# iammadab/zk

Hardware: AMD Instinct MI355X
Metric: field-ops/sec (MLE fold, 2^24 evals, BN254 Fr) + sumcheck prover wall-clock (higher is better)
Workload: dtype u256 (8 x u32 Montgomery limbs, integer)

## Files before the change

zk_amd/csrc/capi.hip:

```cpp
#include <hip/hip_runtime.h>
#include <sched.h>

#include <algorithm>
#include <array>
#include <atomic>
#include <chrono>
#include <condition_variable>
#include <mutex>
#include <cstdio>
#include <map>
#include <new>
#include <set>
#include <string>
#include <thread>
#include <utility>
#include <vector>

#include "../../include/zk_amd.h"
#include "host_core.hpp"
#include "copy_helpers.hpp"
#include "prover_state.hpp"
#include "env.hpp"
#include "kernels.cuh"
#include "eval_kernels.cuh"
// ... 77 lines not shown
        case ZK_ERR_VERIFY_ROUNDS: return "invalid proof: require 1 round poly for each variable in poly";
        case ZK_ERR_VERIFY_SUM: return "verifier check failed: claimed_sum != p(0) + p(1)";
        case ZK_ERR_COEFF_RANGE: return "coefficient map represents more than specificed number of variables";
        case ZK_ERR_PANIC_INVERSE: return "reference panics: (x_i - x_j).inverse().unwrap() on a repeated x (interpolate_xy)";
        case ZK_ERR_EVAL_ASSIGNMENT: return "evaluate requires an assignment for every variable";
        case ZK_ERR_SELECTOR_LEN: return "the selector array len should be the same as the number of variables";
        case ZK_ERR_SELECTOR_SINGLE: return "only select single variable, cannot get indexes for constant or multiple variables";
        case ZK_ERR_BAD_ARG: return "bad argument";
        case ZK_ERR_BAD_FIELD: return "unknown field id";
        case ZK_ERR_NO_DEVICE: return "no usable gfx950 device (libzk_amd has no CPU fallback)";
        case ZK_ERR_HIP: return "HIP runtime error (see zk_last_hip_error)";
        case ZK_ERR_ALLOC: return "allocation failed";
        case ZK_ERR_UNSUPPORTED: return "unsupported configuration";
        case ZK_ERR_CONTEXT_MISMATCH: return "handle belongs to a different context";
        case ZK_ERR_GKR_REJECT: return "gkr verifier check failed: layer wiring / input claim mismatch";
        case ZK_ERR_COMM: return "collective failed (see zk_last_hip_error)";
        default: return "unknown status";
    }
}
extern "C" const char *zk_last_hip_error(void) { return g_hip_err.c_str(); }

extern "C" int32_t zk_device_count(int32_t *out) {
    if (!out) return ZK_ERR_BAD_ARG;
    int n = 0;
    if (hipGetDeviceCount(&n) != hipSuccess) n = 0;
    *out = n;
    return ZK_OK;
}

extern "C" int32_t zk_field_modulus(int32_t field, uint64_t out[4]) {
    const uint64_t *m = field_modulus_limbs(field);
    if (!m || !out) return m ? ZK_ERR_BAD_ARG : ZK_ERR_BAD_FIELD;
    memcpy(out, m, 32);
    return ZK_OK;
}
extern "C" int32_t zk_field_two_adicity(int32_t field, int32_t *out) {
    const FieldInfo *fi = field_info(field);
    if (!fi) return ZK_ERR_BAD_FIELD;
    if (!out) return ZK_ERR_BAD_ARG;
    *out = (int32_t)fi->two_adicity;
    return ZK_OK;
}
extern "C" int32_t zk_field_root_of_unity(int32_t field, uint64_t log_n, uint64_t out[4]) {
    const FieldInfo *fi = field_info(field);
    if (!fi) return ZK_ERR_BAD_FIELD;
    if (!out) return ZK_ERR_BAD_ARG;
    Fe w;
    if (log_n > 64 || !field_root_of_unity(*fi, (uint32_t)log_n, w)) return ZK_ERR_FFT_NO_ROOT;
    fe_to_u64limbs(w, out);
    return ZK_OK;
}
extern "C" int32_t zk_fe_from_u64(int32_t field, uint64_t v, uint64_t out[4]) {
    const FieldInfo *fi = field_info(field);
    if (!fi) return ZK_ERR_BAD_FIELD;
    uint64_t l[4] = {v, 0, 0, 0};
    fe_to_u64limbs(fe_from_canonical(fe_from_u64limbs(l), fi->P), out);
    return ZK_OK;
}
extern "C" int32_t zk_fe_from_canonical(int32_t field, const uint64_t limbs[4], uint64_t out[4]) {
    const FieldInfo *fi = field_info(field);
    if (!fi) return ZK_ERR_BAD_FIELD;
    Fe c = fe_from_u64limbs(limbs), d;
    if (!sub8(d.v, c.v, fi->P.p)) return ZK_ERR_BAD_ARG;
    fe_to_u64limbs(fe_from_canonical(c, fi->P), out);
    return ZK_OK;
}
extern "C" int32_t zk_fe_to_canonical(int32_t field, const uint64_t a[4], uint64_t out[4]) {
    const FieldInfo *fi = field_info(field);
    if (!fi) return ZK_ERR_BAD_FIELD;
    fe_to_u64limbs(fe_to_canonical(fe_from_u64limbs(a), fi->P), out);
    return ZK_OK;
}
extern "C" int32_t zk_fe_from_be_bytes_mod_order(int32_t field, const uint8_t *bytes, size_t len, uint64_t out[4]) {
    const FieldInfo *fi = field_info(field);
    if (!fi) return ZK_ERR_BAD_FIELD;
    fe_to_u64limbs(fe_from_be_bytes_mod_order(bytes, len, fi->P), out);
    return ZK_OK;
}

static int32_t ctx_init_device(zk_ctx *c) {
    HIPCHK(hipSetDevice(c->device));
    HIPCHK(hipStreamCreateWithFlags(&c->own_stream, hipStreamNonBlocking));
    c->stream = c->own_stream;
    HIPCHK(hipMalloc(&c->d_partials, (size_t)kMaxGrid * kMaxSums * 32));
    HIPCHK(hipMalloc(&c->d_sums, (size_t)kMaxSums * 32 * 3));
    HIPCHK(hipHostMalloc(&c->h_pinned, (size_t)kMaxSums * 32 * 3, kPolledHostFlags));
    HIPCHK(hipHostMalloc((void **)&c->h_flag, 64 * kMaxBatch, kPolledHostFlags));
    memset(c->h_flag, 0, 64 * kMaxBatch);
    HIPCHK(hipEventCreate(&c->ev0));
    HIPCHK(hipEventCreate(&c->ev1));
    return ZK_OK;
}
static void ctx_teardown(zk_ctx *c) {
    (void)hipSetDevice(c->device);
    if (c->own_stream) (void)hipStreamSynchronize(c->stream);
    for (auto &kv : c->twiddles) (void)hipFree(kv.second);
    for (auto &kv : c->lagrange_w) (void)hipFree(kv.second);
    for (auto &kv : c->ntt_plans) {
        (void)hipFree((void *)kv.second.w_lo);
        (void)hipFree((void *)kv.second.w_hi);
        for (int p = 0; p < 4; ++p)
            if (kv.second.w_full[p]) (void)hipFree((void *)kv.second.w_full[p]);
    }
    pool_trim(c);
    (void)hipFree(c->d_partials);
    (void)hipFree(c->d_sums);
    if (c->h_pinned) (void)hipHostFree(c->h_pinned);
    if (c->h_flag) (void)hipHostFree(c->h_flag);
    if (c->h_results) (void)hipHostFree(c->h_results);
    for (int b = 0; b < 2; ++b) {
        if (c->h_absorb[b]) (void)hipHostFree(c->h_absorb[b]);
        if (c->ev_absorb[b]) (void)hipEventDestroy(c->ev_absorb[b]);
    }
    if (c->ev0) (void)hipEventDestroy(c->ev0);
    if (c->ev1) (void)hipEventDestroy(c->ev1);
    if (c->own_stream) (void)hipStreamDestroy(c->own_stream);
    delete c;
}
extern "C" int32_t zk_ctx_create(int32_t field, int32_t device, zk_ctx **out) {
    if (!out) return ZK_ERR_BAD_ARG;
    const FieldInfo *fi = field_info(field);
    if (!fi) return ZK_ERR_BAD_FIELD;
    int n = 0;
    if (hipGetDeviceCount(&n) != hipSuccess || n <= 0 || device < 0 || device >= n) return ZK_ERR_NO_DEVICE;
    hipDeviceProp_t prop;
    if (hipGetDeviceProperties(&prop, device) != hipSuccess) return ZK_ERR_NO_DEVICE;
    if (std::string(prop.gcnArchName).find("gfx950") == std::string::npos) return ZK_ERR_NO_DEVICE;
    zk_ctx *c = new (std::nothrow) zk_ctx();
    if (!c) return ZK_ERR_ALLOC;
    c->field = field;
    c->device = device;
    c->fi = fi;
    c->own_stream = c->stream = nullptr;
    c->ev0 = c->ev1 = nullptr;
    c->d_partials = c->d_sums = c->h_pinned = nullptr;
    c->h_flag = nullptr;
    c->flag_seq = 0;
    c->h_results = nullptr;
    c->h_results_bytes = 0;
    c->pool_bytes = c->pool_checked = 0;
    c->inv2 = fe_inverse(fe_from_u32(2, fi->P), fi->P);
    c->pipe_consts.inv2p = mul29_prepare(c->inv2, fi->P);
    {
        Fe v = {{1, 0, 0, 0, 0, 0, 0, 0}};
        for (int i = 0; i < 266; ++i) v = fe_add(v, v, fi->P);
        split29(v.v, c->pipe_consts.k266.l);
    }
    c->d_dbg = nullptr;
    c->dbg_launch = 0;
    c->h_absorb[0] = c->h_absorb[1] = nullptr;
    c->h_absorb_bytes = 0;
    c->ev_absorb[0] = c->ev_absorb[1] = nullptr;
    const int32_t rc = ctx_init_device(c);
    if (rc != ZK_OK) {
        ctx_teardown(c);
        return rc;
    }
    *out = c;
    return ZK_OK;
}
extern "C" int32_t zk_ctx_destroy(zk_ctx *c) {
    if (!c) return ZK_OK;
    ctx_teardown(c);
    return ZK_OK;
}
extern "C" int32_t zk_ctx_synchronize(zk_ctx *c) {
    if (!c) return ZK_ERR_BAD_ARG;
// ... 647 lines not shown
    if (f[0]->ctx != c) return ZK_ERR_CONTEXT_MISMATCH;
    if (k > (uint64_t)kMaxFactors) return ZK_ERR_UNSUPPORTED;
    return use_device(c);
}

extern "C" int32_t zk_prod_reduce(zk_ctx *c, const zk_mle *const *f, uint64_t k, zk_mle **out) {
    if (!out) return ZK_ERR_BAD_ARG;
    ZKCHK(product_args(c, f, k));
    zk_mle *o = nullptr;
    ZKCHK(mle_alloc(c, f[0]->n_vars, &o));
    FactorPtrs fp = {};
    for (uint64_t i = 0; i < k; ++i) fp.in[i] = f[i]->d;
    const uint64_t n = 1ull << f[0]->n_vars;
    if (n >= 64) {
        uint64_t g = n / kBlock;
        if (g > 2 * kMaxGridStream) g = 2 * kMaxGridStream;
        k_prod_reduce_run<<<(uint32_t)(g ? g : 1), kBlock, 0, c->stream>>>(fp, (int)k, n, o->d, c->fi->P);
    } else {
        k_prod_reduce<<<grid_for(n), kBlock, 0, c->stream>>>(fp, (int)k, n, o->d, c->fi->P);
    }
    HIPCHK(hipGetLastError());
    *out = o;
    return ZK_OK;
}

extern "C" int32_t zk_product_evaluate(zk_ctx *c, const zk_mle *const *f, uint64_t k, const uint64_t *point,
                                       uint64_t n_point, uint64_t out[4]) {
    if (!out || (!point && n_point)) return ZK_ERR_BAD_ARG;
    ZKCHK(product_args(c, f, k));
    if (n_point != f[0]->n_vars) return ZK_ERR_EVAL_ARITY;
    Fe prod = fe_one(c->fi->P);
    for (uint64_t i = 0; i < k; ++i) {
        uint64_t v[4];
        ZKCHK(zk_mle_evaluate(c, f[i], point, n_point, v));
        prod = fe_mul(prod, fe_from_u64limbs(v), c->fi->P);
    }
    fe_to_u64limbs(prod, out);
    return ZK_OK;
}

static inline uint64_t *epart_counters(uint64_t *d_epart) { return d_epart + 2 * (kEpartBytes / 8); }
static int32_t scratch_alloc(zk_ctx *c, ProverScratch &ps, uint64_t rounds, uint32_t D, const DeviceChain *chain = nullptr) {
    ps = ProverScratch{};
    ps.rp_bytes = (size_t)(rounds ? rounds : 1) * (D + 1) * 32;
    ps.ch_bytes = (size_t)(rounds ? rounds : 1) * 32;
    if (chain) {
        ps.external = true;
        ps.d_sponge = chain->d_sponge;
        ps.d_rp = chain->d_rp;
        ps.d_ch = chain->d_ch;
        ps.d_final = chain->d_final;
        ps.d_epart = chain->d_epart;
    } else {
        ZKCHK(ps.sponge_block.alloc(c, sizeof(WordSponge)));
        ps.d_sponge = ps.sponge_block.as<WordSponge>();
    }
    ZKCHK(ps.chal_block.alloc(c, kChalBlockBytes));
    ps.d_challenge = ps.chal_block.as();
    ps.d_claim = ps.d_challenge + 2 * kChalWords;
    if (chain) return ZK_OK;
    ZKCHK(ps.epart_block.alloc(c, kEpartBlockBytes));
    ps.d_epart = ps.epart_block.as();
    ZKCHK(ps.proof_block.alloc(c, ps.proof_block_bytes()));
    ps.d_rp = ps.proof_block.as();
    ps.d_ch = ps.d_rp + ps.rp_bytes / 8;
    ps.d_final = ps.d_ch + ps.ch_bytes / 8;
    return ZK_OK;
}
int32_t zk::results_staging(zk_ctx *c, size_t bytes, uint8_t **out) {
    if (c->h_results_bytes < bytes) {
        if (c->h_results) (void)hipHostFree(c->h_results);
        c->h_results = nullptr;
        c->h_results_bytes = 0;
        size_t cap = 1 << 16;
        while (cap < bytes) cap <<= 1;
        HIPCHK(hipHostMalloc((void **)&c->h_results, cap, kPolledHostFlags));
        c->h_results_bytes = cap;
    }
    *out = c->h_results;
    return ZK_OK;
}

static inline uint64_t partials_capacity() { return g_batch ? (uint64_t)kMaxGrid * kMaxSums / kMaxBatch : (uint64_t)kMaxGrid * kMaxSums; }
static inline uint64_t *partials_of(zk_ctx *c) { return g_batch ? c->d_partials + (size_t)g_batch->cur * partials_capacity() * 4 : c->d_partials; }
static inline RoundLaunchCtx launch_ctx(zk_ctx *c) {
    RoundLaunchCtx lc = {c->stream, &c->fi->P, partials_of(c), partials_capacity(), {}};
    return lc;
}
static int32_t launch_tail(zk_ctx *c, uint32_t nblocks, uint32_t ns, WordSponge *sponge, uint64_t *out_rp, uint64_t *out_ch, uint64_t *d_challenge,
                           uint64_t *lanes, const TailDerive &dv, const PendingSponge *init = nullptr) {
    const uint64_t *part = partials_of(c);
    hipStream_t st = c->stream;
    const FieldParams *P = &c->fi->P;
    if (init && init->valid && sponge == init->dst && !lanes && !g_batch) {
        k_round_tail_init<<<1, kBlock, 0, st>>>(part, nblocks, ns, sponge, out_rp, out_ch, d_challenge, *P, dv, init->w, init->zero2);
        HIPCHK(hipGetLastError());
        return ZK_OK;
    }
    if (init && init->valid) {
        k_store_sponge<<<1, 64, 0, st>>>(init->w, init->dst, init->zero2);
        HIPCHK(hipGetLastError());
    }
    auto single = [=]() {
        k_round_tail<<<1, kBlock, 0, st>>>(part, nblocks, ns, sponge, out_rp, out_ch, d_challenge, lanes, *P, dv);
        return hipGetLastError();
    };
    if (!lanes && batch_record(BK_TAIL, 0, 1, kBlock, 0, nblocks, ns, 0, 0, TailSlot{part, sponge, out_rp, out_ch, d_challenge, dv}, single)) return ZK_OK;
    HIPCHK(single());
    return ZK_OK;
}
int32_t zk::launch_reduce_tail(zk_ctx *c, uint32_t nblocks, uint32_t ns, uint64_t *out_rp) {
    k_round_tail<<<1, kBlock, 0, c->stream>>>(c->d_partials, nblocks, ns, nullptr, out_rp, nullptr, nullptr, nullptr, c->fi->P);
    HIPCHK(hipGetLastError());
    return ZK_OK;
}
static bool claim_in_round() {
    static const bool v = env_u64("ZK_CLAIM_IN_ROUND", 1, 0, 1) != 0;
    return v;
}
static inline bool fast_degree(uint32_t D) { return D >= 1 && D <= 4; }

struct TailTargets {
    WordSponge *sponge;
    uint64_t *out_rp;
    uint64_t *out_ch;
    uint64_t *d_challenge;
    uint64_t *lanes;
    const PendingSponge *init;
    uint64_t *claim_park;
    TailDerive *lanes_dv;
};
static std::vector<Fe> interp_weights_compute(uint32_t D, const FieldParams &P) {
    std::vector<Fe> w(D + 1);
    for (uint32_t i = 0; i <= D; ++i) {
        Fe den = fe_one(P);
        const Fe xi = fe_from_u32(i, P);
        for (uint32_t j = 0; j <= D; ++j)
            if (j != i) den = fe_mul(den, fe_sub(xi, fe_from_u32(j, P), P), P);
        w[i] = fe_inverse(den, P);
    }
    return w;
}
static std::vector<Fe> interp_weights(uint32_t D, const FieldParams &P) {
    static std::mutex mu;
    static std::map<std::pair<std::array<uint32_t, 8>, uint32_t>, std::vector<Fe>> cache;
    std::array<uint32_t, 8> key;
    for (int i = 0; i < 8; ++i) key[i] = P.p[i];
    std::lock_guard<std::mutex> lock(mu);
    auto it = cache.find({key, D});
    if (it == cache.end()) it = cache.emplace(std::make_pair(key, D), interp_weights_compute(D, P)).first;
    return it->second;
}
static uint64_t skip1_min_pairs() {
    static const uint64_t v = env_u64("ZK_SKIP1_MIN_PAIRS", (uint64_t)1 << 16, 1, (uint64_t)1 << 40);
    return v;
}
static inline TermSpec single_term(int k) {
    TermSpec ts = {1, {k, 0, 0, 0}};
    return ts;
}
struct DeferredTail {
    uint32_t blocks;
    bool skip1;
    bool lead;
    const uint64_t *claim;
};
static uint64_t lead_min_pairs() {
    static const uint64_t v = env_u64("ZK_LEAD_MIN_PAIRS", (uint64_t)1 << 16, 1, (uint64_t)1 << 40);
    return v;
}
static bool shard_skip_on() {
    static const bool v = env_u64("ZK_SHARD_SKIP1", 1, 0, 1) != 0;
    return v;
}
static int32_t launch_sums(zk_ctx *c, const FactorPtrs &fp, const TermSpec &ts, uint64_t q, uint32_t D, bool fused,
                           const uint64_t *d_r, const TailTargets &tt, const TailDerive *dv = nullptr, DeferredTail *defer = nullptr) {
    if (defer) defer->blocks = 0;
    const FieldParams &P = c->fi->P;
    if (fast_degree(D)) {
        uint32_t total = 0;
        int first = 0;
        const bool may_derive = !tt.lanes || (tt.lanes_dv && shard_skip_on());
        bool skip1 = dv && dv->prev_rp && tt.claim_park && fused && may_derive && D <= (uint32_t)kMaxSkipDegree && q >= skip1_min_pairs();
        bool lead = may_derive && q >= lead_min_pairs();
        ClaimJob cjob = {};
        if (skip1 && claim_in_round()) cjob = ClaimJob{dv->prev_rp, dv->prev_chal, dv->w, tt.claim_park, D + 1};
        auto with_claim = [&](RoundLaunchCtx lc) {
            lc.claim = cjob;
            return lc;
        };
        auto tail_dv = [&]() {
            TailDerive t = skip1 && dv ? *dv : TailDerive{};
            t.lead = lead ? D : 0;
            t.claim = (t.prev_rp && cjob.out) ? cjob.out : nullptr;
            if (tt.lanes) {
                if (tt.lanes_dv) *tt.lanes_dv = t;
                t.local_only = 1;
            }
            return t;
        };
        if (tt.lanes_dv) *tt.lanes_dv = TailDerive{};
        if (ts.n_terms == 2 && ts.term_k[1] == 1) {
            uint32_t g = 0;
            const int lrc = launch_round_plus1(with_claim(launch_ctx(c)), fp, ts.term_k[0], q, D, fused, d_r, &g, &skip1, &lead);
            if (lrc == kLaunchHipError) {
                g_hip_err = "round kernel launch failed";
                return ZK_ERR_HIP;
            }
            if (lrc == kLaunchOk) {
                if (defer) {
                    defer->blocks = g;
                    defer->skip1 = skip1;
                    defer->claim = skip1 ? cjob.out : nullptr;
                    defer->lead = lead;
                    return ZK_OK;
                }
                return launch_tail(c, g, D + 1, tt.sponge, tt.out_rp, tt.out_ch, tt.d_challenge, tt.lanes, tail_dv(), tt.init);
            }
        }
        if (ts.n_terms != 1) {
            skip1 = lead = false;
            cjob = {};
        }
        for (int i = 0; i < ts.n_terms; ++i) {
            FactorPtrs sub = {};
            for (int f = 0; f < ts.term_k[i]; ++f) {
                sub.in[f] = fp.in[first + f];
                sub.out[f] = fp.out[first + f];
            }
            RoundLaunchCtx lc = with_claim(launch_ctx(c));
            lc.d_partials += (size_t)total * (D + 1) * 4;
            lc.capacity_elems -= (uint64_t)total * (D + 1);
            uint32_t g = 0;
            const int lrc = launch_round(lc, sub, ts.term_k[i], q, D, fused, d_r, &g, &skip1, &lead);
            if (lrc == kLaunchUnsupported) return ZK_ERR_UNSUPPORTED;
            if (lrc != kLaunchOk) {
                g_hip_err = "round kernel launch failed";
                return ZK_ERR_HIP;
            }
            total += g;
            first += ts.term_k[i];
        }
        if (defer) {
            defer->blocks = total;
            defer->skip1 = skip1;
            defer->claim = skip1 ? cjob.out : nullptr;
            defer->lead = lead;
            return ZK_OK;
        }
        return launch_tail(c, total, D + 1, tt.sponge, tt.out_rp, tt.out_ch, tt.d_challenge, tt.lanes, tail_dv(), tt.init);
    }
    if (ts.n_terms != 1) return ZK_ERR_UNSUPPORTED;
    const int k = ts.term_k[0];
    for (uint32_t t = 0; t <= D; ++t) {
        uint32_t g = 0;
        if (launch_round_single_t(launch_ctx(c), fp, k, q, fe_from_u32(t, P), &g) != kLaunchOk) {
            g_hip_err = "round kernel launch failed";
            return ZK_ERR_HIP;
        }
        k_round_tail<<<1, kBlock, 0, c->stream>>>(c->d_partials, g, 1, nullptr, c->d_sums + 4 * t, nullptr, nullptr, nullptr, P);
        HIPCHK(hipGetLastError());
    }
    k_round_tail<<<1, kBlock, 0, c->stream>>>(c->d_sums, 1, D + 1, tt.sponge, tt.out_rp, tt.out_ch, tt.d_challenge, tt.lanes, P);
    HIPCHK(hipGetLastError());
    return ZK_OK;
}

extern "C" int32_t zk_round_sums(zk_ctx *c, const zk_mle *const *f, uint64_t k, uint32_t D, uint64_t *out) {
    if (!out) return ZK_ERR_BAD_ARG;
    ZKCHK(product_args(c, f, k));
    if (D >= kMaxSums) return ZK_ERR_UNSUPPORTED;
    if (f[0]->n_vars == 0) return ZK_ERR_PANIC_INDEX;
    FactorPtrs fp = {};
    for (uint64_t i = 0; i < k; ++i) fp.in[i] = f[i]->d;
    const uint64_t q = 1ull << (f[0]->n_vars - 1);
    uint64_t *d_out = c->d_sums + 4 * kMaxSums;
    TailTargets tt = {nullptr, d_out, nullptr, nullptr, nullptr, nullptr, nullptr};
    ZKCHK(launch_sums(c, fp, single_term((int)k), q, D, false, nullptr, tt));
    HIPCHK(hipMemcpyAsync(out, d_out, (size_t)(D + 1) * 32, hipMemcpyDeviceToHost, c->stream));
    HIPCHK(hipStreamSynchronize(c->stream));
    return ZK_OK;
}

extern "C" int32_t zk_transcript_new(zk_transcript **out) {
    if (!out) return ZK_ERR_BAD_ARG;
    zk_transcript *t = new (std::nothrow) zk_transcript();
    if (!t) return ZK_ERR_ALLOC;
    t->sp.init();
    *out = t;
    return ZK_OK;
}
extern "C" int32_t zk_transcript_free(zk_transcript *t) {
    delete t;
    return ZK_OK;
}
extern "C" int32_t zk_transcript_append(zk_transcript *t, const uint8_t *data, size_t len) {
    if (!t || (!data && len)) return ZK_ERR_BAD_ARG;
    t->sp.update(data, len);
    return ZK_OK;
}
extern "C" int32_t zk_transcript_sample_challenge(zk_transcript *t, uint8_t out[32]) {
    if (!t || !out) return ZK_ERR_BAD_ARG;
    t->sp.sample_challenge(out);
    return ZK_OK;
}
extern "C" int32_t zk_transcript_sample_field_element(zk_transcript *t, int32_t field, uint64_t out[4]) {
    if (!t || !out) return ZK_ERR_BAD_ARG;
    const FieldInfo *fi = field_info(field);
    if (!fi) return ZK_ERR_BAD_FIELD;
    uint8_t h[32];
    t->sp.sample_challenge(h);
    fe_to_u64limbs(fe_from_be_bytes_mod_order(h, 32, fi->P), out);
    return ZK_OK;
}
extern "C" int32_t zk_transcript_sample_n_field_elements(zk_transcript *t, int32_t field, uint64_t n, uint64_t *out) {
    if (!t || (!out && n)) return ZK_ERR_BAD_ARG;
    if (!field_info(field)) return ZK_ERR_BAD_FIELD;
    for (uint64_t i = 0; i < n; ++i) ZKCHK(zk_transcript_sample_field_element(t, field, out + 4 * i));
    return ZK_OK;
}
extern "C" int32_t zk_keccak256(const uint8_t *data, size_t len, uint8_t out[32]) {
    if ((!data && len) || !out) return ZK_ERR_BAD_ARG;
    Sponge s;
    s.init();
    s.update(data, len);
    s.finalize_reset(out);
    return ZK_OK;
}

void zk::absorb_elements(Sponge &sp, const uint64_t *elems, uint64_t n, const FieldParams &P) {
// ... 225 lines not shown
    int k, extra;
    if (!pipe_limit_pairs() || !pipe_shape(st, &k, &extra)) return false;
    if (m_s < 3) return false;
    if (!finish_pipe_on() && m_s - 1 <= (uint64_t)kFinishVars) return false;
    return ((uint64_t)1 << (m_s - 2)) <= pipe_limit_pairs();
}
static int32_t finish_pipe_enqueue(RoundState &st) {
    zk_ctx *c = st.c;
    int k = 0, extra = 0;
    (void)pipe_shape(st, &k, &extra);
    FinishPipeLaunch fl = {};
    fl.k = k;
    fl.extra = extra;
    fl.D = st.D;
    fl.m_in = (uint32_t)st.vars_left;
    fl.entry = st.pipe_active ? 2 : (st.pending_fold ? 1 : 0);
    fl.e_partials = epart_of_round(st, st.round);
    fl.e_blocks = 1;
    if (st.pipe_active && !st.pipe_total) {
        fl.e_partials += (size_t)pipe_values_per_block(k, st.D) * 4;
        fl.e_blocks = st.pipe_blocks;
    }
    fl.pc = c->pipe_consts;
    fl.chal_in = chal_prev(st);
    const uint64_t remaining = st.pending_fold ? st.vars_left - 1 : st.vars_left;
    fl.chal_last = chal_of_round(st, st.round + remaining - 1);
    fl.sponge = st.ps.d_sponge;
    fl.out_rp = st.ps.d_rp + st.round * (st.D + 1) * 4;
    fl.out_ch = st.ps.d_ch + st.round * 4;
    fl.out_final = st.d_final;
    fl.dbg = pipe_dbg_slot(c, true);
    fl.pub = st.pub;
    FactorPtrs fp = {};
    for (uint64_t i = 0; i < st.k; ++i) fp.in[i] = st.cur[i];
    const int lrc = launch_finish_pipe(launch_ctx(c), fp, fl);
    if (lrc != kLaunchOk) {
        g_hip_err = "pipelined finisher launch failed";
        return lrc == kLaunchUnsupported ? ZK_ERR_UNSUPPORTED : ZK_ERR_HIP;
    }
    st.round += remaining;
    st.vars_left = 0;
    st.pending_fold = false;
    st.pipe_active = false;
    st.published = st.pub.flag != nullptr;
    return ZK_OK;
}
static PipeTailArgs pipe_tail_args(const RoundState &st, int mode, const uint64_t *partials, uint32_t nblocks, uint32_t n_in) {
    PipeTailArgs ta = {};
    ta.dbg = pipe_dbg_slot(st.c, false);
    ta.partials = partials;
    ta.nblocks = nblocks;
    ta.n_in = n_in;
    ta.mode = mode;
    ta.chal_in = chal_prev(st);
    ta.chal_out = chal_cur(st);
    ta.sponge = st.ps.d_sponge;
    ta.out_rp = st.ps.d_rp + st.round * (st.D + 1) * 4;
    ta.out_ch = st.ps.d_ch + st.round * 4;
    ta.pc = st.c->pipe_consts;
    return ta;
}
static int32_t pipe_enter(RoundState &st, const DeferredTail &dt) {
    zk_ctx *c = st.c;
    int k = 0, extra = 0;
    (void)pipe_shape(st, &k, &extra);
    PipeLaunch pl = {};
    pl.k = k;
    pl.extra = extra;
    pl.D = st.D;
    pl.fold = false;
    pl.emit = 1;
    pl.q = (uint64_t)1 << (st.vars_left - 2);
    pl.chal_fold = nullptr;
    pl.e_partials = epart_of_round(st, st.round + 1);
    pl.done_counter = epart_counter(st, st.round + 1);
    pl.tail = pipe_tail_args(st, 0, partials_of(c), dt.blocks, st.D + 1);
    if (dt.skip1) {
        pl.tail.dv = st.dv;
        pl.tail.dv.prev_rp = pl.tail.out_rp - (size_t)(st.D + 1) * 4;
        pl.tail.dv.prev_chal = chal_prev(st);
        pl.tail.dv.claim = dt.claim;
    }
    pl.tail.dv.lead = dt.lead ? st.D : 0;
    FactorPtrs fp = {};
    for (uint64_t i = 0; i < st.k; ++i) fp.in[i] = fp.out[i] = st.cur[i];
    uint32_t g = 0;
    const int lrc = launch_round_pipe(launch_ctx(c), fp, pl, &g);
    if (lrc != kLaunchOk) {
        g_hip_err = "pipelined round launch failed";
        return lrc == kLaunchUnsupported ? ZK_ERR_UNSUPPORTED : ZK_ERR_HIP;
    }
    st.pipe_active = true;
    st.pipe_blocks = g;
    st.pipe_total = true;
    return ZK_OK;
}
static int32_t pipe_step(RoundState &st) {
    zk_ctx *c = st.c;
    int k = 0, extra = 0;
    (void)pipe_shape(st, &k, &extra);
    const uint64_t m = st.vars_left;
    const bool stay = pipe_wants_next(st, m - 1);
    PipeLaunch pl = {};
    pl.k = k;
    pl.extra = extra;
    pl.D = st.D;
    pl.fold = true;
    pl.emit = stay ? 1 : 0;
    pl.q = m >= 3 ? (uint64_t)1 << (m - 3) : 0;
    if (pl.q == 0) return ZK_ERR_BAD_ARG;
    pl.chal_fold = chal_prev(st);
    pl.e_partials = epart_of_round(st, st.round + 1);
    pl.done_counter = epart_counter(st, st.round + 1);
    pl.tail = pipe_tail_args(st, 1, epart_of_round(st, st.round), 1, pipe_values_per_block(k, st.D));
    if (!st.pipe_total) {
        pl.tail.partials = epart_of_round(st, st.round) + (size_t)pipe_values_per_block(k, st.D) * 4;
        pl.tail.nblocks = st.pipe_blocks;
    }
    FactorPtrs fp = {};
    for (uint64_t i = 0; i < st.k; ++i) {
        fp.in[i] = st.cur[i];
        fp.out[i] = (st.first_out_of_place && st.scratch[i]) ? st.scratch[i].as() : st.cur[i];
    }
    uint32_t g = 0;
    const int lrc = launch_round_pipe(launch_ctx(c), fp, pl, &g);
    if (lrc != kLaunchOk) {
        g_hip_err = "pipelined round launch failed";
        return lrc == kLaunchUnsupported ? ZK_ERR_UNSUPPORTED : ZK_ERR_HIP;
    }
    for (uint64_t i = 0; i < st.k; ++i) st.cur[i] = fp.out[i];
    st.first_out_of_place = false;
    st.vars_left = m - 1;
    st.pipe_active = stay;
    st.pipe_blocks = g;
    st.pipe_total = true;
    ++st.round;
    return ZK_OK;
}

template <int K, int D>
static int32_t launch_finish(zk_ctx *c, const FactorPtrs &fp, uint32_t m_in, int pending, uint64_t *d_challenge, WordSponge *sp,
                             uint64_t *out_rp, uint64_t *out_ch, uint64_t *out_final) {
    const uint32_t m = pending ? m_in - 1 : m_in;
    const size_t lds = (size_t)K * ((size_t)32 << m) + (kBlock / 64) * (D + 1) * 32 + (D + 1) * 32 + 48;
    HIPCHK(hipFuncSetAttribute(reinterpret_cast<const void *>(&k_finish<K, D>), hipFuncAttributeMaxDynamicSharedMemorySize, (int)lds));
    hipStream_t st = c->stream;
    const FieldParams *P = &c->fi->P;
    auto single = [=]() {
        k_finish<K, D><<<1, kBlock, lds, st>>>(fp, m_in, pending, *P, d_challenge, sp, out_rp, out_ch, out_final);
        return hipGetLastError();
    };
    if (batch_record_other(single)) return ZK_OK;
    HIPCHK(single());
    return ZK_OK;
}
static bool finish_shape_ok(uint64_t k, uint32_t D) {
    const int shape = (int)k * 10 + (int)D;
    return shape == 11 || shape == 12 || shape == 21 || shape == 22 || shape == 23 || shape == 32 || shape == 33;
}
static int32_t finish_enqueue(RoundState &st) {
    zk_ctx *c = st.c;
    FactorPtrs fp = {};
    for (uint64_t i = 0; i < st.k; ++i) fp.in[i] = st.cur[i];
    const int pending = st.pending_fold ? 1 : 0;
    const uint32_t m_in = (uint32_t)st.vars_left;
    const uint64_t remaining = pending ? st.vars_left - 1 : st.vars_left;
    uint64_t *out_rp = st.ps.d_rp + st.round * (st.D + 1) * 4, *out_ch = st.ps.d_ch + st.round * 4;
    int32_t rc = ZK_ERR_UNSUPPORTED;
    if (st.terms.n_terms > 1) {
        const uint32_t m = pending ? m_in - 1 : m_in;
        const size_t lds = (size_t)st.k * ((size_t)32 << m) + (kBlock / 64) * (st.D + 1) * 32 + (st.D + 1) * 32 + 48;
        const FieldParams &P = c->fi->P;
#define ZK_FINISH_TERMS(DD)                                                                                                     \
    case DD:                                                                                                                    \
        if (hipFuncSetAttribute(reinterpret_cast<const void *>(&k_finish_terms<DD>), hipFuncAttributeMaxDynamicSharedMemorySize, \
                                (int)lds) != hipSuccess)                                                                        \
            return ZK_ERR_HIP;                                                                                                  \
        k_finish_terms<DD><<<1, kBlock, lds, c->stream>>>(fp, st.terms, m_in, pending, P, chal_prev(st), st.ps.d_sponge,     \
                                                          out_rp, out_ch, st.d_final);                                          \
        break;
        switch (st.D) {
            ZK_FINISH_TERMS(1)
            ZK_FINISH_TERMS(2)
            ZK_FINISH_TERMS(3)
            ZK_FINISH_TERMS(4)
            default: return ZK_ERR_UNSUPPORTED;
        }
#undef ZK_FINISH_TERMS
        rc = hipGetLastError() == hipSuccess ? ZK_OK : ZK_ERR_HIP;
    } else {
        switch ((int)st.k * 10 + (int)st.D) {
            case 11: rc = launch_finish<1, 1>(c, fp, m_in, pending, chal_prev(st), st.ps.d_sponge, out_rp, out_ch, st.d_final); break;
            case 12: rc = launch_finish<1, 2>(c, fp, m_in, pending, chal_prev(st), st.ps.d_sponge, out_rp, out_ch, st.d_final); break;
            case 21: rc = launch_finish<2, 1>(c, fp, m_in, pending, chal_prev(st), st.ps.d_sponge, out_rp, out_ch, st.d_final); break;
            case 22: rc = launch_finish<2, 2>(c, fp, m_in, pending, chal_prev(st), st.ps.d_sponge, out_rp, out_ch, st.d_final); break;
            case 23: rc = launch_finish<2, 3>(c, fp, m_in, pending, chal_prev(st), st.ps.d_sponge, out_rp, out_ch, st.d_final); break;
            case 32: rc = launch_finish<3, 2>(c, fp, m_in, pending, chal_prev(st), st.ps.d_sponge, out_rp, out_ch, st.d_final); break;
            case 33: rc = launch_finish<3, 3>(c, fp, m_in, pending, chal_prev(st), st.ps.d_sponge, out_rp, out_ch, st.d_final); break;
            default: break;
        }
    }
    if (rc == ZK_OK) {
        st.round += remaining;
        st.vars_left = 0;
        st.pending_fold = false;
    }
    return rc;
}
static inline bool finish_applies(const RoundState &st) {
    if (st.terms.n_terms == 1 ? !finish_shape_ok(st.k, st.D) : !fast_degree(st.D)) return false;
    const uint64_t after = st.pending_fold ? st.vars_left - 1 : st.vars_left;
    return after >= 1 && after <= (uint64_t)kFinishVars;
}

static int32_t prover_step(RoundState &st, bool *finished_in_kernel) {
    if (st.init.valid && (finish_pipe_applies(st) || st.pipe_active || finish_applies(st))) ZKCHK(flush_pending_sponge(st));
    if (finish_pipe_applies(st)) {
        *finished_in_kernel = true;
        return finish_pipe_enqueue(st);
    }
    if (st.pipe_active) return pipe_step(st);
    if (finish_applies(st)) {
        *finished_in_kernel = true;
        return finish_enqueue(st);
    }
    const uint64_t m_s = st.pending_fold ? st.vars_left - 1 : st.vars_left;
    DeferredTail dt = {0, false, false, nullptr};
    const bool enter = fast_degree(st.D) && pipe_wants_next(st, m_s);
    ZKCHK(round_enqueue(st, nullptr, enter ? &dt : nullptr));
    if (enter && dt.blocks) ZKCHK(pipe_enter(st, dt));
    ++st.round;
    return ZK_OK;
}

int32_t zk::sponge_to_device(zk_ctx *c, const Sponge &host, WordSponge *d_sponge, uint64_t *d_epart) {
    WordSponge w;
    if (!w.from_byte_sponge(host)) return ZK_ERR_BAD_ARG;
    uint64_t *zero2 = d_epart ? epart_counters(d_epart) : nullptr;
    hipStream_t st = c->stream;
    auto single = [=]() {
        k_store_sponge<<<1, 64, 0, st>>>(w, d_sponge, zero2);
        return hipGetLastError();
    };
    if (batch_record(BK_STORE_SPONGE, 0, 1, 64, 0, 0, 0, 0, 0, SpongeSlot{w, d_sponge, zero2}, single)) return ZK_OK;
    HIPCHK(single());
    return ZK_OK;
}

static bool has_duplicate_handles(zk_mle *const *f, uint64_t k) {
    for (uint64_t i = 0; i < k; ++i)
        for (uint64_t j = i + 1; j < k; ++j)
            if (f[i] == f[j]) return true;
    return false;
}
int32_t zk::prove_core(zk_ctx *c, zk_mle *const *f, uint64_t k, const TermSpec &ts, uint32_t D, const uint64_t sum[4],
                          int32_t absorb_table, int32_t consume, uint64_t *out_rp, uint64_t *out_ch, uint64_t *out_final,
                          uint64_t *d_keep_ch, uint64_t *d_keep_final, const Sponge *init, const DeviceChain *chain) {
    if (!sum && !chain) return ZK_ERR_BAD_ARG;
    ZKCHK(product_args(c, (const zk_mle *const *)f, k));
    if (chain) {
        const uint64_t n = f[0]->n_vars;
        if (n == 0 || D >= kMaxSums) return ZK_ERR_UNSUPPORTED;
        if (has_duplicate_handles(f, k)) consume = 0;
        RoundState st;
        ZKCHK(round_state_init(st, c, f, k, D, consume != 0, n, chain));
        st.terms = ts;
        st.d_final = st.ps.d_final;
        bool fin = false;
        while (st.round < n) ZKCHK(prover_step(st, &fin));
        if (!fin) {
            FactorPtrs fp = {};
            for (uint64_t i = 0; i < k; ++i) fp.in[i] = st.cur[i];
            k_final_evals<<<1, 64, 0, c->stream>>>(fp, (uint32_t)k, chal_prev(st), st.d_final, c->fi->P);
            HIPCHK(hipGetLastError());
        }
        return ZK_OK;
    }
    if (f[0]->n_vars && (!out_rp || !out_ch)) return ZK_ERR_BAD_ARG;
    if (D >= kMaxSums) return ZK_ERR_UNSUPPORTED;
    const FieldParams &P = c->fi->P;
    const uint64_t n = f[0]->n_vars;
    Sponge sp;
    if (init) sp = *init;
    else sp.init();
    if (absorb_table) ZKCHK(absorb_tables(c, sp, f, k));
    absorb_elements(sp, sum, 1, P);
    if (n == 0) {
        if (out_final)
            for (uint64_t i = 0; i < k; ++i) ZKCHK(zk_mle_download(c, f[i], out_final + 4 * i));
        return ZK_OK;
    }
    if (has_duplicate_handles(f, k)) consume = 0;
    static const bool host_dbg = env_flag("ZK_HOST_DEBUG");
    const auto t_enter = std::chrono::steady_clock::now();
    RoundState st;
    ZKCHK(round_state_init(st, c, f, k, D, consume != 0, n));
    st.terms = ts;
    if (out_final) st.d_final = st.ps.d_final;
    uint8_t *stage = nullptr;
    const size_t block = st.ps.proof_block_bytes();
    uint32_t seq = 0;
    auto enqueue = [&]() -> int32_t {
        static const bool sponge_in_tail = env_u64("ZK_SPONGE_IN_TAIL", 1, 0, 1) != 0;
        if (sponge_in_tail && !g_batch) {
            if (!st.init.w.from_byte_sponge(sp)) return ZK_ERR_BAD_ARG;
            st.init.dst = st.ps.d_sponge;
            st.init.zero2 = st.ps.d_epart ? epart_counters(st.ps.d_epart) : nullptr;
            st.init.valid = true;
        } else {
            ZKCHK(sponge_to_device(c, sp, st.ps.d_sponge, st.ps.d_epart));
// ... 670 lines not shown
```

zk_amd/csrc/common.cuh:

```cuda
#pragma once
#include "field.cuh"

namespace zk {

constexpr int kBlock = 256;
constexpr int kMaxFactors = 8;

struct FactorPtrs {
    const uint64_t *in[kMaxFactors];
    uint64_t *out[kMaxFactors];
};

constexpr int kMaxBatch = 8;
template <class Slot>
struct BatchOf {
    Slot a[kMaxBatch];
};
struct FactorPtrs4 {
    const uint64_t *in[4];
    uint64_t *out[4];
};
ZK_HD FactorPtrs4 factor_ptrs4(const FactorPtrs &f) {
    FactorPtrs4 r;
    for (int i = 0; i < 4; ++i) r.in[i] = f.in[i], r.out[i] = f.out[i];
// ... 11 lines not shown
struct TermSpec {
    int n_terms;
    int term_k[kMaxTerms];
};
#if defined(__HIPCC__)
ZK_D Mul29 load_challenge29c(const uint64_t *rptr) {
    const uint32_t *w = reinterpret_cast<const uint32_t *>(rptr) + kChalCanonWord;
    Mul29 r;
#pragma unroll
    for (int i = 0; i < 9; ++i) r.l[i] = __builtin_amdgcn_readfirstlane(w[i]);
    return r;
}
ZK_D Mul29 load_challenge29(const uint64_t *rptr) {
    const uint32_t *w = reinterpret_cast<const uint32_t *>(rptr) + 8;
    Mul29 r;
#pragma unroll
    for (int i = 0; i < 9; ++i) r.l[i] = __builtin_amdgcn_readfirstlane(w[i]);
    return r;
}
typedef uint32_t u32x4_t __attribute__((ext_vector_type(4)));
ZK_D uint4 nt_load16(const uint4 *p) {
    const u32x4_t v = __builtin_nontemporal_load(reinterpret_cast<const u32x4_t *>(p));
    return make_uint4(v.x, v.y, v.z, v.w);
}
ZK_D void nt_store16(uint4 v, uint4 *p) {
    const u32x4_t w = {v.x, v.y, v.z, v.w};
    __builtin_nontemporal_store(w, reinterpret_cast<u32x4_t *>(p));
}
ZK_D uint32_t swap_pair_lane(uint32_t v) { return __builtin_amdgcn_mov_dpp(v, 0xB1 , 0xF, 0xF, true); }
ZK_D Fe pair_gather(const uint4 &A, const uint4 &B, bool odd) {
    const uint4 send = odd ? A : B;
    const uint4 recv = make_uint4(swap_pair_lane(send.x), swap_pair_lane(send.y), swap_pair_lane(send.z), swap_pair_lane(send.w));
    Fe r;
    if (!odd) r = {{A.x, A.y, A.z, A.w, recv.x, recv.y, recv.z, recv.w}};
    else r = {{recv.x, recv.y, recv.z, recv.w, B.x, B.y, B.z, B.w}};
    return r;
}
ZK_D void pair_scatter(const Fe &e, bool odd, uint4 &A, uint4 &B) {
    const uint4 lo = make_uint4(e.v[0], e.v[1], e.v[2], e.v[3]), hi = make_uint4(e.v[4], e.v[5], e.v[6], e.v[7]);
    const uint4 send = odd ? lo : hi;
    const uint4 recv = make_uint4(swap_pair_lane(send.x), swap_pair_lane(send.y), swap_pair_lane(send.z), swap_pair_lane(send.w));
    if (!odd) {
        A = lo;
        B = recv;
    } else {
        A = recv;
        B = hi;
    }
}
ZK_D uint32_t pair_owned(uint32_t lane) { return (lane >> 1) + ((lane & 1) << 5); }
ZK_D Fe run_load(const uint64_t *run , uint32_t lane) {
    const uint4 *p = reinterpret_cast<const uint4 *>(run) + lane;
    return pair_gather(p[0], p[64], lane & 1);
}
ZK_D void run_store(uint64_t *run, uint32_t lane, const Fe &e) {
    uint4 A, B;
    pair_scatter(e, lane & 1, A, B);
    uint4 *p = reinterpret_cast<uint4 *>(run) + lane;
    p[0] = A;
    p[64] = B;
}

ZK_D Fe run_load_nt(const uint64_t *run, uint32_t lane) {
    const uint4 *p = reinterpret_cast<const uint4 *>(run) + lane;
    return pair_gather(nt_load16(p), nt_load16(p + 64), lane & 1);
}
ZK_D void run_store_nt(uint64_t *run, uint32_t lane, const Fe &e) {
    uint4 A, B;
    pair_scatter(e, lane & 1, A, B);
    uint4 *p = reinterpret_cast<uint4 *>(run) + lane;
    nt_store16(A, p);
    nt_store16(B, p + 64);
}

constexpr int kMaxSkipDegree = 4;
struct TailDerive {
    const uint64_t *prev_rp;
    const uint64_t *prev_chal;
    const uint64_t *w;
    uint32_t lead;
    uint32_t local_only;
    const uint64_t *claim;
    uint32_t log_world;
};
struct ClaimJob {
    const uint64_t *prev_rp;
    const uint64_t *prev_chal;
    const uint64_t *w;
    uint64_t *out;
    uint32_t ns;
};
ZK_HD Fe lead_rebuild(uint32_t D, const Fe *S, const FieldParams &P) {
    const Fe L = S[D];
    if (D == 1) return fe_add(S[0], L, P);
    if (D == 2) {
        const Fe a = fe_add(S[1], L, P);
        return fe_sub(fe_add(a, a, P), S[0], P);
    }
    Fe b = fe_add(fe_sub(S[2], S[1], P), fe_add(L, L, P), P);
    b = fe_add(fe_add(b, b, P), b, P);
    return fe_add(S[0], b, P);
}

template <int CTRL>
ZK_D Fe fe_dpp(const Fe &s) {
    Fe o;
#pragma unroll
    for (int i = 0; i < 8; ++i) o.v[i] = __builtin_amdgcn_update_dpp(0u, s.v[i], CTRL, 0xF, 0xF, true);
    return o;
}
ZK_D Fe fe_wave_sum(Fe s, const FieldParams &P, uint32_t width = 64) {
    if (width > 32) {
        Fe a, b;
#pragma unroll
        for (int i = 0; i < 8; ++i) {
            const auto r = __builtin_amdgcn_permlane32_swap(s.v[i], s.v[i], false, false);
            a.v[i] = r[0];
            b.v[i] = r[1];
        }
        s = fe_add(a, b, P);
    }
    if (width > 16) {
        Fe a, b;
#pragma unroll
        for (int i = 0; i < 8; ++i) {
            const auto r = __builtin_amdgcn_permlane16_swap(s.v[i], s.v[i], false, false);
            a.v[i] = r[0];
            b.v[i] = r[1];
        }
        s = fe_add(a, b, P);
    }
    if (width > 8) s = fe_add(s, fe_dpp<0x128>(s), P);
    if (width > 4) s = fe_add(s, fe_dpp<0x12C>(s), P);
    if (width > 2) s = fe_add(s, fe_dpp<0x12E>(s), P);
    if (width > 1) s = fe_add(s, fe_dpp<0x12F>(s), P);
    return s;
}
ZK_D Fe claim_eval(const ClaimJob &cj, const FieldParams &P) {
    const uint32_t lane = threadIdx.x & 63;
    const Fe r = fe_load(cj.prev_chal, 0);
    Fe term = fe_zero();
    if (lane < cj.ns) {
        Fe one;
#pragma unroll
        for (int i = 0; i < 8; ++i) one.v[i] = P.r1[i];
        term = fe_mul(fe_load(cj.prev_rp, lane), fe_load(cj.w, lane), P);
        Fe node = fe_zero();
        for (uint32_t u = 0; u < cj.ns; ++u) {
            if (u != lane) term = fe_mul(term, fe_sub(r, node, P), P);
            node = fe_add(node, one, P);
        }
    }
    return fe_wave_sum(term, P, 8);
}

constexpr int kEvalHighMax = 12;
struct EvalHighPoint {
    uint32_t n;
    uint32_t r[kEvalHighMax][8];
};
ZK_D uint32_t eval_high_lane(uint32_t n) { return n > 8 ? 15u : n > 4 ? 7u : n > 2 ? 3u : n > 1 ? 1u : 0u; }
ZK_D Fe eval_high_weight(const EvalHighPoint &ph, uint64_t g, uint32_t lane, const FieldParams &P) {
    Fe one;
#pragma unroll
    for (int i = 0; i < 8; ++i) one.v[i] = P.r1[i];
    Fe f = one;
    for (uint32_t k = 0; k < ph.n; ++k) {
        Fe r;
#pragma unroll
        for (int i = 0; i < 8; ++i) r.v[i] = ph.r[k][i];
        const Fe sel = (g >> k) & 1 ? r : fe_sub(one, r, P);
        if ((lane & 15) == k) f = sel;
    }
    if (ph.n > 8) f = fe_mul(f, fe_dpp<0x128>(f), P);
    if (ph.n > 4) f = fe_mul(f, fe_dpp<0x124>(f), P);
    if (ph.n > 2) f = fe_mul(f, fe_dpp<0x122>(f), P);
    if (ph.n > 1) f = fe_mul(f, fe_dpp<0x121>(f), P);
    return f;
}
#endif

}
```

zk_amd/csrc/field.cuh:

```cuda
#pragma once
#include <stdint.h>

#if defined(__HIPCC__)
#include <hip/hip_runtime.h>
#define ZK_HD __host__ __device__ __forceinline__
#define ZK_D __device__ __forceinline__
#else
#define ZK_HD inline
#define ZK_D inline
#endif

namespace zk {

struct FieldParams {
    uint32_t p[8];
    uint32_t r1[8];
    uint32_t r2[8];
    uint32_t inv;
    uint32_t bits;
    uint32_t p29[9];
    uint32_t inv29;
    uint32_t r2_29[9];
    uint32_t r2s_29[9];
};
// ... 275 lines not shown
    return fe_mul(x, r2, P);
}
ZK_HD Fe fe_to_canonical(const Fe &a, const FieldParams &P) {
    uint32_t t[16];
#pragma unroll
    for (int i = 0; i < 8; ++i) {
        t[i] = a.v[i];
        t[i + 8] = 0;
    }
    return redc(t, P);
}
ZK_HD Fe fe_from_u32(uint32_t x, const FieldParams &P) {
    Fe v = {{x, 0, 0, 0, 0, 0, 0, 0}};
    return fe_from_canonical(v, P);
}

template <int KMAX>
ZK_HD void ladder9(uint32_t s[9], const FieldParams &P) {
#pragma unroll
    for (int k = KMAX; k >= 0; --k) {
        uint32_t d[9];
        uint32_t borrow = 0;
#pragma unroll
        for (int i = 0; i < 9; ++i) {
            uint32_t pk;
            if (k == 0) pk = (i < 8) ? P.p[i] : 0u;
            else pk = ((i < 8) ? (P.p[i] << k) : 0u) | ((i > 0) ? (P.p[i - 1] >> (32 - k)) : 0u);
            uint32_t bo;
            d[i] = __builtin_subc(s[i], pk, borrow, &bo);
            borrow = bo;
        }
#pragma unroll
        for (int i = 0; i < 9; ++i) s[i] = borrow ? s[i] : d[i];
    }
}

struct WideAcc {
    uint32_t v[17];
};
ZK_HD void wide_zero(WideAcc &w) {
#pragma unroll
    for (int i = 0; i < 17; ++i) w.v[i] = 0;
}
template <int C>
ZK_HD void wide_mac_col(WideAcc &w, Acc &acc, const uint32_t a[8], const uint32_t b[8]) {
    constexpr int lo = C < 8 ? 0 : C - 7, hi = C < 8 ? C : 7;
    acc_add32(acc, w.v[C]);
    mac_col<hi - lo + 1>(acc, a + lo, b + (C - lo));
    w.v[C] = acc_shift(acc);
    if constexpr (C + 1 < 15) wide_mac_col<C + 1>(w, acc, a, b);
}
ZK_HD void wide_mac(WideAcc &w, const uint32_t a[8], const uint32_t b[8]) {
    Acc acc = {0, 0};
    wide_mac_col<0>(w, acc, a, b);
    acc_add32(acc, w.v[15]);
    w.v[15] = acc_shift(acc);
    w.v[16] += (uint32_t)acc.lh;
}
constexpr int kMaxLazy = 32;
ZK_HD Fe redc_wide(const WideAcc &w, const FieldParams &P) {
    uint32_t m[8];
    Acc acc = {0, 0};
    uint32_t s[9];
    redc_cols<0>(w.v, m, s, acc, P);
    s[8] = (uint32_t)acc.lh;
    {
        uint64_t c = 0;
        const uint32_t top = w.v[16];
#pragma unroll
        for (int i = 0; i < 8; ++i) {
            c += (uint64_t)top * P.r1[i] + s[i];
            s[i] = (uint32_t)c;
            c >>= 32;
        }
        s[8] += (uint32_t)c;
    }
    ladder9<4>(s, P);
    Fe r;
#pragma unroll
    for (int i = 0; i < 8; ++i) r.v[i] = s[i];
    return r;
}

ZK_HD Fe fe_reduce_u256(const uint32_t x[8], const FieldParams &P) {
    uint32_t s[9];
#pragma unroll
    for (int i = 0; i < 8; ++i) s[i] = x[i];
    s[8] = 0;
    ladder9<4>(s, P);
    Fe r;
#pragma unroll
    for (int i = 0; i < 8; ++i) r.v[i] = s[i];
    return r;
}

struct Mul29 {
    uint32_t l[9];
};
ZK_HD void split29(const uint32_t a[8], uint32_t out[9]) {
    constexpr uint32_t M = (1u << 29) - 1;
#pragma unroll
    for (int i = 0; i < 9; ++i) {
        const int bit = 29 * i, w = bit >> 5, sh = bit & 31;
        uint32_t v = a[w] >> sh;
        if (sh > 3 && w + 1 < 8) v |= a[w + 1] << (32 - sh);
        out[i] = (i < 8) ? (v & M) : v;
    }
}
ZK_HD Mul29 mul29_prepare(const Fe &c, const FieldParams &P) {
    Fe t = c;
#pragma unroll
    for (int i = 0; i < 5; ++i) t = fe_add(t, t, P);
    Mul29 m;
    split29(t.v, m.l);
    return m;
}
template <bool LAZY = false, bool TWO = false>
ZK_HD Fe mul29_core(const uint32_t (&x)[9], const uint32_t (&y)[9], const Mul29 &c, const FieldParams &P, const Mul29 *c2 = nullptr) {
    constexpr uint32_t M = (1u << 29) - 1;
    uint32_t m[9], r[9];
    uint64_t acc = 0;
#pragma unroll
    for (int k = 0; k < 9; ++k) {
#pragma unroll
        for (int i = 0; i <= k; ++i) acc += (uint64_t)x[i] * c.l[k - i];
        if constexpr (TWO) {
#pragma unroll
            for (int i = 0; i <= k; ++i) acc += (uint64_t)y[i] * c2->l[k - i];
        }
#pragma unroll
        for (int i = 0; i < k; ++i) acc += (uint64_t)m[i] * P.p29[k - i];
        m[k] = ((uint32_t)acc * P.inv29) & M;
        acc += (uint64_t)m[k] * P.p29[0];
        acc >>= 29;
    }
#pragma unroll
    for (int k = 9; k < 17; ++k) {
#pragma unroll
        for (int i = k - 8; i < 9; ++i) acc += (uint64_t)x[i] * c.l[k - i];
        if constexpr (TWO) {
#pragma unroll
            for (int i = k - 8; i < 9; ++i) acc += (uint64_t)y[i] * c2->l[k - i];
        }
#pragma unroll
        for (int i = k - 8; i < 9; ++i) acc += (uint64_t)m[i] * P.p29[k - i];
        r[k - 9] = (uint32_t)acc & M;
        acc >>= 29;
    }
    r[8] = (uint32_t)acc;
    Fe s;
#pragma unroll
    for (int w = 0; w < 8; ++w) {
        const int bit = 32 * w, i = bit / 29, sh = bit - 29 * i;
        uint32_t v = r[i] >> sh;
        v |= r[i + 1] << (29 - sh);
        if (29 - sh + 29 < 32 && i + 2 < 9) v |= r[i + 2] << (58 - sh);
        s.v[w] = v;
    }
    if constexpr (LAZY) return s;
    Fe d, o;
    const uint32_t borrow = sub8(d.v, s.v, P.p);
#pragma unroll
    for (int i = 0; i < 8; ++i) o.v[i] = borrow ? s.v[i] : d.v[i];
    return o;
}
template <bool LAZY = false, bool TWO = false>
// ... 45 lines not shown
```

zk_amd/csrc/host_field.hpp:

```cpp
#pragma once
#include <stdint.h>
#include <string.h>

#include "field.cuh"

namespace zk {

struct FieldInfo {
    FieldParams P;
    uint32_t two_adicity;
    uint32_t generator;
    Fe two_adic_root;
    bool ready;
};

inline const uint64_t *field_modulus_limbs(int field) {
    static const uint64_t M[3][4] = {
        {0x43e1f593f0000001ULL, 0x2833e84879b97091ULL, 0xb85045b68181585dULL, 0x30644e72e131a029ULL},
        {0xffffffff00000001ULL, 0x53bda402fffe5bfeULL, 0x3339d80809a1d805ULL, 0x73eda753299d7d48ULL},
        {0x0a11800000000001ULL, 0x59aa76fed0000001ULL, 0x60b44d1e5c37b001ULL, 0x12ab655e9a2ca556ULL},
    };
    return (field >= 0 && field < 3) ? M[field] : nullptr;
}

inline Fe fe_from_u64limbs(const uint64_t l[4]) {
    Fe r;
    for (int i = 0; i < 4; ++i) {
        r.v[2 * i] = (uint32_t)l[i];
        r.v[2 * i + 1] = (uint32_t)(l[i] >> 32);
    }
    return r;
}
inline void fe_to_u64limbs(const Fe &a, uint64_t l[4]) {
    for (int i = 0; i < 4; ++i) l[i] = (uint64_t)a.v[2 * i] | ((uint64_t)a.v[2 * i + 1] << 32);
}

inline Fe fe_pow_limbs(const Fe &x, const uint32_t e[8], const FieldParams &P) {
    Fe acc = fe_one(P);
    for (int i = 255; i >= 0; --i) {
        acc = fe_sqr(acc, P);
        if ((e[i / 32] >> (i % 32)) & 1u) acc = fe_mul(acc, x, P);
    }
    return acc;
}
inline Fe fe_pow_u64(const Fe &x, uint64_t e, const FieldParams &P) {
    Fe acc = fe_one(P), base = x;
    while (e) {
        if (e & 1) acc = fe_mul(acc, base, P);
        base = fe_sqr(base, P);
        e >>= 1;
    }
    return acc;
}
inline Fe fe_inverse(const Fe &a, const FieldParams &P) {
    uint32_t e[8], two[8] = {2, 0, 0, 0, 0, 0, 0, 0};
    sub8(e, P.p, two);
    return fe_pow_limbs(a, e, P);
}

inline const FieldInfo *field_info(int field) {
    static FieldInfo info[3];
    static const uint32_t adicity[3] = {28, 32, 47};
    static const uint32_t gen[3] = {5, 7, 22};
    if (field < 0 || field > 2) return nullptr;
    FieldInfo &I = info[field];
    if (I.ready) return &I;
    FieldParams &P = I.P;
    Fe pm = fe_from_u64limbs(field_modulus_limbs(field));
    memcpy(P.p, pm.v, 32);
    uint32_t x = 1;
    for (int i = 0; i < 5; ++i) x *= 2u - P.p[0] * x;
    P.inv = 0u - x;
    int top = 7;
    while (top > 0 && P.p[top] == 0) --top;
    P.bits = 32 * top + (32 - __builtin_clz(P.p[top]));
    uint32_t v[8] = {1, 0, 0, 0, 0, 0, 0, 0}, d[8];
    for (int i = 0; i < 512; ++i) {
        uint32_t c = add8(v, v, v);
        uint32_t b = sub8(d, v, P.p);
        if (c | (b ^ 1u)) memcpy(v, d, 32);
        if (i == 255) memcpy(P.r1, v, 32);
    }
    memcpy(P.r2, v, 32);
    split29(P.p, P.p29);
    P.inv29 = P.inv & ((1u << 29) - 1);
    {
        Fe r2;
        memcpy(r2.v, P.r2, 32);
        const Mul29 k0 = mul29_prepare(r2, P);
        Fe r2s = r2;
        for (int i = 0; i < 5; ++i) r2s = fe_add(r2s, r2s, P);
        const Mul29 k1 = mul29_prepare(r2s, P);
        memcpy(P.r2_29, k0.l, sizeof k0.l);
        memcpy(P.r2s_29, k1.l, sizeof k1.l);
    }
    {
        const int rp_log = 257 - (int)P.bits;
        int lazy_log = 0;
        while ((1 << lazy_log) < kMaxLazy) ++lazy_log;
        const int top_log = lazy_log + 2 * (int)P.bits - 512;
        const uint64_t rp = rp_log >= 0 && rp_log < 32 ? (1ull << rp_log) : ~0ull;
        const uint64_t top = top_log < 0 ? 0 : (top_log < 32 ? (1ull << top_log) : ~0ull);
        if (rp_log < 0 || rp + 1 + top >= 32 || rp + 1 + top < rp) return nullptr;
    }
    I.two_adicity = adicity[field];
    I.generator = gen[field];
    uint32_t t[8], one[8] = {1, 0, 0, 0, 0, 0, 0, 0};
    sub8(t, P.p, one);
    for (uint32_t s = 0; s < I.two_adicity; ++s) {
        for (int i = 0; i < 7; ++i) t[i] = (t[i] >> 1) | (t[i + 1] << 31);
        t[7] >>= 1;
    }
    I.two_adic_root = fe_pow_limbs(fe_from_u32(I.generator, P), t, P);
    I.ready = true;
    return &I;
}

inline bool field_root_of_unity(const FieldInfo &I, uint32_t log_n, Fe &out) {
    if (log_n > I.two_adicity) return false;
    Fe w = I.two_adic_root;
    for (uint32_t i = log_n; i < I.two_adicity; ++i) w = fe_sqr(w, I.P);
    out = w;
    return true;
}

inline void fe_to_bytes_be(const Fe &a, const FieldParams &P, uint8_t out[32]) {
    Fe c = fe_to_canonical(a, P);
    for (int i = 0; i < 8; ++i)
        for (int b = 0; b < 4; ++b) out[31 - (4 * i + b)] = (uint8_t)(c.v[i] >> (8 * b));
}
inline Fe fe_from_be_bytes_mod_order(const uint8_t *bytes, size_t len, const FieldParams &P) {
    Fe acc = fe_zero();
    const Fe c256 = fe_from_u32(256, P);
    for (size_t i = 0; i < len; ++i) acc = fe_add(fe_mul(acc, c256, P), fe_from_u32(bytes[i], P), P);
    return acc;
}

}
```

zk_amd/csrc/kernels.cuh:

```cuda
#pragma once
#include "common.cuh"
#include "keccak.hpp"
#include "transcript.cuh"

namespace zk {

ZK_D uint64_t insert_zero_bit(uint64_t val, uint32_t pos) {
    const uint64_t low = val & ((1ull << pos) - 1ull);
    return ((val >> pos) << (pos + 1)) | low;
}

__global__ __launch_bounds__(kBlock) void k_fold(const uint64_t *in, uint64_t *out,
                                                 uint64_t pairs, uint32_t pos, FieldParams P, Mul29 r) {
    const uint64_t stride = (uint64_t)gridDim.x * kBlock;
    for (uint64_t j = (uint64_t)blockIdx.x * kBlock + threadIdx.x; j < pairs; j += stride) {
        const uint64_t l = insert_zero_bit(j, pos);
        const Fe lo = fe_load(in, l);
        const Fe hi = fe_load(in, l | (1ull << pos));
        const Fe d = fe_sub(lo, hi, P);
        fe_store(out, j, fe_sub(lo, fe_mul29(d, r, P), P));
    }
}

__global__ __launch_bounds__(kBlock) void k_fold_msb(const uint64_t *in, uint64_t *out, uint64_t half, FieldParams P, Mul29 r) {
// ... 256 lines not shown
    }
}

__global__ __launch_bounds__(kBlock) void k_prod_reduce_run(FactorPtrs fp, int k, uint64_t n, uint64_t *__restrict__ out, FieldParams P) {
    const uint32_t lane = threadIdx.x & 63;
    const bool odd = lane & 1;
    const uint64_t wave = ((uint64_t)blockIdx.x * kBlock + threadIdx.x) >> 6;
    const uint64_t nwaves = ((uint64_t)gridDim.x * kBlock) >> 6;
    uint4 *out4 = reinterpret_cast<uint4 *>(out);
    for (uint64_t e0 = wave * 64; e0 < n; e0 += nwaves * 64) {
        const uint64_t c0 = 2 * e0 + lane;
        Fe acc;
        {
            const uint4 *q = reinterpret_cast<const uint4 *>(fp.in[0]);
            acc = pair_gather(nt_load16(q + c0), nt_load16(q + c0 + 64), odd);
        }
        for (int f = 1; f < k; ++f) {
            const uint4 *q = reinterpret_cast<const uint4 *>(fp.in[f]);
            acc = fe_mul_tt(acc, pair_gather(nt_load16(q + c0), nt_load16(q + c0 + 64), odd), P);
        }
        uint4 oa, ob;
        pair_scatter(acc, odd, oa, ob);
        nt_store16(oa, out4 + c0);
        nt_store16(ob, out4 + c0 + 64);
    }
}
__global__ __launch_bounds__(kBlock) void k_prod_reduce(FactorPtrs fp, int k, uint64_t n, uint64_t *__restrict__ out,
                                                        FieldParams P) {
    const uint64_t stride = (uint64_t)gridDim.x * kBlock;
    for (uint64_t j = (uint64_t)blockIdx.x * kBlock + threadIdx.x; j < n; j += stride) {
        Fe acc = fe_load(fp.in[0], j);
        for (int f = 1; f < k; ++f) acc = fe_mul(acc, fe_load(fp.in[f], j), P);
        fe_store(out, j, acc);
    }
}

ZK_D LaneSponge lane_sponge_from_arg(const WordSponge &w, const LaneKeccak &L) {
    LaneSponge sp;
    sp.a = 0;
#pragma unroll
    for (int i = 0; i < 25; ++i)
        if (L.index == i) sp.a = w.s[i];
    sp.pos = w.pos;
    return sp;
}
ZK_D void round_tail_body(const uint64_t *__restrict__ partials, uint32_t nblocks, uint32_t ns, WordSponge *__restrict__ sponge,
                          uint64_t *__restrict__ out_rp, uint64_t *__restrict__ out_ch, uint64_t *__restrict__ d_challenge,
                          uint64_t *__restrict__ lanes, const FieldParams &P, const TailDerive &dv, const WordSponge *init = nullptr,
                          uint64_t *__restrict__ zero2 = nullptr) {
    __shared__ Fe fin[256];
    __shared__ Fe claim;
    const int lane = threadIdx.x & 63, wave = threadIdx.x >> 6;
    const bool wave0 = __builtin_amdgcn_readfirstlane(wave) == 0;
    const bool derive1 = dv.prev_rp != nullptr;
    const LaneKeccak L = lane_keccak_init();
    LaneSponge sp = {0, 0};
    if (sponge && wave0) sp = init ? lane_sponge_from_arg(*init, L) : lane_sponge_load(sponge, L);
    if (init && zero2 && threadIdx.x >= 64 && threadIdx.x < 66) zero2[threadIdx.x - 64] = 0;
    for (uint32_t t = wave; t < ns; t += kBlock / 64) {
        if (derive1 && t == 1 && (dv.claim || dv.local_only)) {
            if (lane == 0) {
                if (dv.local_only) fin[1] = fe_zero();
                else claim = fe_load(dv.claim, 0);
            }
            continue;
        }
        if (derive1 && t == 1) {
            const Fe r = fe_load(dv.prev_chal, 0);
            Fe term = fe_zero();
            if ((uint32_t)lane < ns) {
                Fe one;
#pragma unroll
                for (int i = 0; i < 8; ++i) one.v[i] = P.r1[i];
                const Fe wt = fe_load(dv.w, lane);
                term = fe_mul(fe_load(dv.prev_rp, lane), wt, P);
                Fe node = fe_zero();
                for (uint32_t u = 0; u < ns; ++u) {
                    if (u != (uint32_t)lane) term = fe_mul(term, fe_sub(r, node, P), P);
                    node = fe_add(node, one, P);
                }
            }
            term = fe_wave_sum(term, P, 8);
            if (lane == 0) claim = term;
            continue;
        }
        Fe s = fe_zero();
        for (uint32_t b = lane; b < nblocks; b += 8 * 64) {
            Fe x[8];
#pragma unroll
            for (int u = 0; u < 8; ++u) x[u] = b + u * 64 < nblocks ? fe_load(partials, (uint64_t)(b + u * 64) * ns + t) : fe_zero();
            const Fe lo = fe_add(fe_add(x[0], x[1], P), fe_add(x[2], x[3], P), P), hi = fe_add(fe_add(x[4], x[5], P), fe_add(x[6], x[7], P), P);
            s = fe_add(s, fe_add(lo, hi, P), P);
        }
        s = fe_wave_sum(s, P);
        if (lane == 0) fin[t] = s;
    }
    __syncthreads();
    if ((derive1 || dv.lead) && !dv.local_only) {
        if (threadIdx.x == 0) {
            if (derive1) fin[1] = fe_sub(claim, fin[0], P);
            if (dv.lead) fin[dv.lead] = lead_rebuild(dv.lead, fin, P);
        }
        __syncthreads();
    }
    if (threadIdx.x == kBlock - 64) {
        for (uint32_t t = 0; t < ns; ++t) {
            if (out_rp) fe_store(out_rp, t, fin[t]);
            if (lanes)
                for (int i = 0; i < 8; ++i) lanes[8 * t + i] = (uint64_t)fin[t].v[i];
        }
    }
    if (sponge && wave0) {
        lane_absorb_elems(sp, L, fin, ns, P);
        Mul29 ch29;
        Fe ch;
        challenge_forms(lane_squeeze_x(sp, L), (uint32_t)lane, P, ch29, ch);
        publish_challenge_forms(d_challenge, out_ch, ch, ch29, (uint32_t)lane);
        lane_sponge_store(sponge, sp, L);
    }
}
__global__ __launch_bounds__(kBlock) void k_round_tail(const uint64_t *__restrict__ partials, uint32_t nblocks, uint32_t ns,
                                                       WordSponge *__restrict__ sponge, uint64_t *__restrict__ out_rp,
                                                       uint64_t *__restrict__ out_ch, uint64_t *__restrict__ d_challenge,
                                                       uint64_t *__restrict__ lanes, FieldParams P, TailDerive dv = {}) {
    round_tail_body(partials, nblocks, ns, sponge, out_rp, out_ch, d_challenge, lanes, P, dv);
}
__global__ __launch_bounds__(kBlock) void k_round_tail_init(const uint64_t *__restrict__ partials, uint32_t nblocks, uint32_t ns,
                                                            WordSponge *__restrict__ sponge, uint64_t *__restrict__ out_rp,
                                                            uint64_t *__restrict__ out_ch, uint64_t *__restrict__ d_challenge, FieldParams P,
                                                            TailDerive dv, WordSponge init, uint64_t *__restrict__ zero2) {
    round_tail_body(partials, nblocks, ns, sponge, out_rp, out_ch, d_challenge, nullptr, P, dv, &init, zero2);
}
struct TailSlot {
    const uint64_t *partials;
    WordSponge *sponge;
    uint64_t *out_rp, *out_ch, *d_challenge;
    TailDerive dv;
};
__global__ __launch_bounds__(kBlock) void k_round_tail_b(BatchOf<TailSlot> b, uint32_t nblocks, uint32_t ns, FieldParams P) {
    const TailSlot &a = b.a[blockIdx.y];
    round_tail_body(a.partials, nblocks, ns, a.sponge, a.out_rp, a.out_ch, a.d_challenge, nullptr, P, a.dv);
}

constexpr int kFinishVars = 9;
template <int K, int D>
__global__ __launch_bounds__(kBlock) void k_finish(FactorPtrs fp, uint32_t m_in, int pending, FieldParams P,
                                                   uint64_t *d_challenge, WordSponge *gsponge, uint64_t *out_rp, uint64_t *out_ch,
                                                   uint64_t *out_final) {
    constexpr int NS = D + 1;
    extern __shared__ __attribute__((aligned(16))) unsigned char fin_smem[];
    const uint32_t tid = threadIdx.x, lane = tid & 63, wave = tid >> 6;
    const bool wave0 = __builtin_amdgcn_readfirstlane(wave) == 0;
    uint32_t m = pending ? m_in - 1 : m_in;
    const uint32_t n_elems = 1u << m;
    uint64_t *tab = reinterpret_cast<uint64_t *>(fin_smem);
    unsigned char *carve = fin_smem + (size_t)K * n_elems * 32;
    uint32_t(*red)[NS][8] = reinterpret_cast<uint32_t(*)[NS][8]>(carve);
    Fe *fin = reinterpret_cast<Fe *>(carve + (kBlock / 64) * NS * 32);
    Mul29 *sh_r29p = reinterpret_cast<Mul29 *>(carve + (kBlock / 64) * NS * 32 + NS * 32);
    if (pending) {
        const Mul29 r = load_challenge29(d_challenge);
#pragma unroll
        for (int f = 0; f < K; ++f)
            for (uint32_t j = tid; j < n_elems; j += kBlock) {
                const Fe lo = fe_load(fp.in[f], j), hi = fe_load(fp.in[f], j + n_elems);
                fe_store(tab + (size_t)f * n_elems * 4, j, fe_sub(lo, fe_mul29(fe_sub(lo, hi, P), r, P), P));
// ... 503 lines not shown
```

zk_amd/csrc/launch.hpp:

```cpp
#pragma once
#include <hip/hip_runtime.h>
#include <stdint.h>

#include <cstring>
#include <functional>
#include <type_traits>
#include <vector>

#include "common.cuh"

namespace zk {

enum BatchKernel : int { BK_STORE_SPONGE = 1, BK_ROUND_KD, BK_ROUND0_DOT29, BK_ROUND_QUAD, BK_TAIL, BK_PIPE, BK_FINISH_PIPE, BK_OTHER };
struct BatchRecord {
    int kernel;
    uint32_t shape;
    uint32_t grid, block;
    size_t lds;
    uint64_t s[4];
    std::function<hipError_t()> single;
    alignas(16) unsigned char slot[384];
};
struct BatchRecorder {
    int n = 0;
    int cur = 0;
    hipStream_t stream = nullptr;
    const FieldParams *P = nullptr;
    std::vector<BatchRecord> recs[kMaxBatch];
    uint64_t merged = 0, replayed = 0;
};
extern thread_local BatchRecorder *g_batch;
template <class Slot, class F>
inline bool batch_record(int kernel, uint32_t shape, uint32_t grid, uint32_t block, size_t lds, uint64_t s0, uint64_t s1, uint64_t s2, uint64_t s3,
                         const Slot &slot, F &&single) {
    BatchRecorder *r = g_batch;
    if (!r) return false;
    static_assert(sizeof(Slot) <= sizeof(BatchRecord::slot), "slot does not fit a batch record");
    static_assert(std::is_trivially_copyable<Slot>::value, "slots are plain data");
    r->recs[r->cur].emplace_back();
    BatchRecord &rec = r->recs[r->cur].back();
    rec.kernel = kernel;
    rec.shape = shape;
    rec.grid = grid;
    rec.block = block;
    rec.lds = lds;
    rec.s[0] = s0, rec.s[1] = s1, rec.s[2] = s2, rec.s[3] = s3;
    rec.single = std::function<hipError_t()>(std::forward<F>(single));
    std::memcpy(rec.slot, &slot, sizeof(Slot));
    return true;
}
template <class F>
inline bool batch_record_other(F &&single) {
    struct Nothing {
        int x;
    } none = {0};
    return batch_record(BK_OTHER, 0, 0, 0, 0, 0, 0, 0, 0, none, std::forward<F>(single));
}
int batch_launch_rounds(const BatchRecorder &r, size_t idx);
int batch_launch_pipe(const BatchRecorder &r, size_t idx);
template <class Slot>
inline void batch_gather(const BatchRecorder &r, size_t idx, BatchOf<Slot> &out) {
    std::memset(&out, 0, sizeof out);
    for (int b = 0; b < r.n; ++b) std::memcpy(&out.a[b], r.recs[b][idx].slot, sizeof(Slot));
}

struct RoundLaunchCtx {
    hipStream_t stream;
    const FieldParams *P;
    uint64_t *d_partials;
    uint64_t capacity_elems;
    ClaimJob claim;
};
enum { kLaunchOk = 0, kLaunchUnsupported = -1, kLaunchHipError = -2 };
int launch_round(const RoundLaunchCtx &lc, const FactorPtrs &fp, int k, uint64_t q, uint32_t D, bool fused,
                 const uint64_t *d_r, uint32_t *out_grid, bool *skip1 = nullptr, bool *lead = nullptr);
int launch_round_plus1(const RoundLaunchCtx &lc, const FactorPtrs &fp, int k, uint64_t q, uint32_t D, bool fused,
                       const uint64_t *d_r, uint32_t *out_grid, bool *skip1 = nullptr, bool *lead = nullptr);
int launch_round_single_t(const RoundLaunchCtx &lc, const FactorPtrs &fp, int k, uint64_t q, const Fe &tval, uint32_t *out_grid);


constexpr uint32_t kPipeMaxWorkBlocks = 256;
}
#include "pipe_args.hpp"
namespace zk {
struct PipeLaunch {
    int k, extra;
    uint32_t D;
    bool fold;
    int emit;
    uint64_t q;
    const uint64_t *chal_fold;
    uint64_t *e_partials;
    uint32_t *done_counter;
    PipeTailArgs tail;
};
bool pipe_shape_ok(int k, uint32_t D, int extra);
uint32_t pipe_values_per_block(int k, uint32_t D);
uint32_t pipe_rows_per_block(int k, uint32_t D, int extra);
uint32_t pipe_work_blocks(int k, uint32_t D, int extra, uint64_t q);
int launch_round_pipe(const RoundLaunchCtx &lc, const FactorPtrs &fp, const PipeLaunch &pl, uint32_t *out_work_blocks);
int launch_spin_us(hipStream_t stream, uint32_t us);
struct FinishPipeLaunch {
    int k, extra;
    uint32_t D;
    uint32_t m_in;
    int entry;
    const uint64_t *e_partials;
    uint32_t e_blocks;
    PipeConsts pc;
    const uint64_t *chal_in;
    uint64_t *chal_last;
    WordSponge *sponge;
    uint64_t *out_rp, *out_ch, *out_final;
    uint64_t *dbg;
    FinishPublish pub;
};
int launch_finish_pipe(const RoundLaunchCtx &lc, const FactorPtrs &fp, const FinishPipeLaunch &fl);
uint32_t finish_pipe_max_vars(int n_factors);

}
```

zk_amd/csrc/pipe_kernels.cuh:

```cuda
#pragma once
#include "common.cuh"
#include "quad.cuh"
#include "transcript.cuh"
#include "pipe_args.hpp"

namespace zk {

constexpr int kPipeNodeZero = 0, kPipeNodeInf = 1, kPipeNodeOne = 2, kPipeNodeMinus = 3;
constexpr int kPipeThreads = 256;
constexpr int kFinishPipeThreads = 256;

template <int K, int D, int EXTRA>
struct PipeShape {
    static_assert(K >= 1 && K <= 3 && D >= 1 && D <= 3 && K + EXTRA <= 4 && (EXTRA == 0 || K >= 2), "shape");
    static constexpr int NF = K + EXTRA, NS = D + 1, NR = K + 1, NE = NS * NR;
};


template <int K, int D, int EXTRA, bool PLAIN>
struct HexCfg {
    static constexpr int NF = K + EXTRA, NS = D + 1, NR = K + 1;
    static constexpr int XW = NR + (PLAIN ? 2 : 0);
    static constexpr int ROW_FE = NF * NS * XW > NF * 4 ? NF * NS * XW : NF * 4;
    static constexpr int ROW_BYTES = ROW_FE * 32;
// ... 190 lines not shown
    const Fe e0c = lds_fe_load(&W.xch[0][t]);
    if constexpr (K == 1) {
        return fe_add(e0c, m1, P);
    } else if constexpr (K == 2) {
        const Fe c1 = fe_sub(fe_sub(e[kPipeNodeOne], e[kPipeNodeZero], P), e[kPipeNodeInf], P);
        return fe_add(e0c, fe_mul29(fe_add(c1, m1, P), rc29, P), P);
    } else {
        const Fe h = lds_fe_load(&W.xch[1][t]), g = lds_fe_load(&W.xch[2][t]);
        const Fe c2 = fe_sub(h, e[kPipeNodeZero], P), c1 = fe_sub(g, e[kPipeNodeInf], P);
        const Fe acc = fe_add(c1, fe_mul29(fe_add(c2, m1, P), rh29, P), P);
        return fe_add(e0c, fe_mul29(acc, rc29, P), P);
    }
}
ZK_D Fe fe_from_canonical29(const Fe &c, const FieldParams &P) {
    Mul29 k0;
#pragma unroll
    for (int i = 0; i < 9; ++i) k0.l[i] = P.r2_29[i];
    return fe_mul29(c, k0, P);
}

ZK_D void fe_store_sc1(uint64_t *base, uint64_t idx, const Fe &r) {
    unsigned long long *q = reinterpret_cast<unsigned long long *>(base + 4 * idx);
#pragma unroll
    for (int i = 0; i < 4; ++i)
        __hip_atomic_store(q + i, (unsigned long long)r.v[2 * i] | ((unsigned long long)r.v[2 * i + 1] << 32), __ATOMIC_RELAXED, __HIP_MEMORY_SCOPE_AGENT);
}
ZK_D Fe fe_load_sc1(const uint64_t *base, uint64_t idx) {
    const unsigned long long *q = reinterpret_cast<const unsigned long long *>(base + 4 * idx);
    Fe r;
#pragma unroll
    for (int i = 0; i < 4; ++i) {
        const unsigned long long w = __hip_atomic_load(q + i, __ATOMIC_RELAXED, __HIP_MEMORY_SCOPE_AGENT);
        r.v[2 * i] = (uint32_t)w;
        r.v[2 * i + 1] = (uint32_t)(w >> 32);
    }
    return r;
}
ZK_D void dbg_stamp(uint64_t *dbg, int slot) {
    if (dbg && (threadIdx.x & 63) == 0) dbg[slot] = wall_clock64();
}

template <bool SC1 = false>
ZK_D void pipe_reduce_partials(const uint64_t *__restrict__ partials, uint32_t nblocks, uint32_t n_in, Fe *red , Fe (*stage)[16] ,
                               const FieldParams &P) {
    const uint32_t tid = threadIdx.x, idx = tid & 15, slice = tid >> 4, lane = tid & 63, wave = tid >> 6;
    Fe s = fe_zero();
    if (idx < n_in) {
        constexpr uint32_t kStep = kPipeThreads / 16;
        for (uint32_t b = slice; b < nblocks; b += 16 * kStep) {
            Fe x[16];
#pragma unroll
            for (int u = 0; u < 16; ++u)
                x[u] = b + u * kStep < nblocks ? (SC1 ? fe_load_sc1(partials, (uint64_t)(b + u * kStep) * n_in + idx) : fe_load(partials, (uint64_t)(b + u * kStep) * n_in + idx))
                                               : fe_zero();
#pragma unroll
            for (int w = 8; w >= 1; w >>= 1)
#pragma unroll
                for (int u = 0; u < w; ++u) x[u] = fe_add(x[u], x[u + w], P);
            s = fe_add(s, x[0], P);
        }
    }
    s = hex_rows_sum(s, P);
    if (lane < 16) stage[wave][lane] = s;
    __syncthreads();
    if (tid < 16) red[tid] = fe_add(fe_add(stage[0][tid], stage[1][tid], P), fe_add(stage[2][tid], stage[3][tid], P), P);
    __syncthreads();
}

template <int K, int D>
ZK_D void pipe_tail_block(const PipeTailArgs &ta, const FieldParams &P) {
    constexpr int NS = D + 1;
    __shared__ Fe red[16];
    __shared__ Fe stage[4][16];
    __shared__ Fe fin[4];
    __shared__ PipeEvalLds W;
    __shared__ int fin_canonical;
    const uint32_t tid = threadIdx.x, lane = tid & 63;
    const bool wave0 = __builtin_amdgcn_readfirstlane(tid >> 6) == 0;
    const LaneKeccak L = lane_keccak_init();
    LaneSponge sp = {0, 0};
    if (wave0) dbg_stamp(ta.dbg, 0);
    if (wave0) sp = lane_sponge_load(ta.sponge, L);
    const uint32_t wave = __builtin_amdgcn_readfirstlane(tid >> 6);
    if (ta.nblocks == 1) {
        if (wave >= 2) return;
        if (wave0 && lane < 16 && lane < ta.n_in) red[lane] = fe_load(ta.partials, lane);
    } else {
        pipe_reduce_partials(ta.partials, ta.nblocks, ta.n_in, red, stage, P);
        if (wave >= 2) return;
    }
    __shared__ Fe digest_x;
    Fe x = fe_zero();
    if (wave0) {
        __builtin_amdgcn_s_setprio(3);
        dbg_stamp(ta.dbg, 1);
        Fe s = fe_zero();
        if (ta.mode == 1) {
            const Mul29 rh29 = load_challenge29(ta.chal_in), rc29 = load_challenge29c(ta.chal_in);
            pipe_eval_consts(W, ta.pc, lane);
            if (lane == 0) pipe_eval_set(W, 0, K == 1 ? rc29 : rh29);
            __builtin_amdgcn_wave_barrier();
            s = pipe_eval_canon<K, D>(red, W, rh29, rc29, lane, P);
        } else {
            s = red[lane < (uint32_t)NS ? lane : 0];
            if (ta.dv.prev_rp && ta.dv.claim) {
                const Fe c0 = fe_load(ta.dv.claim, 0);
                const Fe s0 = red[0];
                if (lane == 1) s = fe_sub(c0, s0, P);
            } else if (ta.dv.prev_rp) {
                const Fe r = fe_load(ta.dv.prev_chal, 0);
                Fe term = fe_zero();
                if (lane < (uint32_t)NS) {
                    const Fe wt = fe_load(ta.dv.w, lane);
                    term = fe_mul(fe_load(ta.dv.prev_rp, lane), wt, P);
                    Fe node = fe_zero();
                    const Fe one = fe_one(P);
                    for (uint32_t u = 0; u < (uint32_t)NS; ++u) {
                        if (u != lane) term = fe_mul(term, fe_sub(r, node, P), P);
                        node = fe_add(node, one, P);
                    }
                }
                const Fe claim = fe_wave_sum(term, P, 8);
                Fe c0;
#pragma unroll
                for (int i = 0; i < 8; ++i) c0.v[i] = __builtin_amdgcn_readfirstlane(claim.v[i]);
                const Fe s0 = red[0];
                if (lane == 1) s = fe_sub(c0, s0, P);
            }
            if (ta.dv.lead) {
                if (lane < (uint32_t)NS) fin[lane] = s;
                __builtin_amdgcn_wave_barrier();
                if (lane == ta.dv.lead) s = lead_rebuild(ta.dv.lead, fin, P);
                __builtin_amdgcn_wave_barrier();
            }
        }
        if (lane < (uint32_t)NS) {
            fin[lane] = s;
            if (ta.mode != 1) fe_store(ta.out_rp, lane, s);
        }
        if (lane == 0) fin_canonical = ta.mode == 1;
        dbg_stamp(ta.dbg, 2);
        if (ta.mode == 1) lane_absorb_elems<true>(sp, L, fin, NS, P);
        else lane_absorb_elems(sp, L, fin, NS, P);
        x = lane_squeeze_x(sp, L);
        if (lane == 0) digest_x = x;
        dbg_stamp(ta.dbg, 3);
    }
    __syncthreads();
    if (wave0) {
        publish_challenge29_both(ta.chal_out, challenge29_both(x, ta.pc.k266, lane, P), lane);
        lane_sponge_store(ta.sponge, sp, L);
        dbg_stamp(ta.dbg, 4);
    } else {
        const bool rp = fin_canonical && lane < (uint32_t)NS;
        const Fe v = fe_from_canonical29(rp ? fin[lane] : digest_x, P);
        if (rp) fe_store(ta.out_rp, lane, v);
        if (lane == 16) {
            fe_store(ta.chal_out, 0, v);
            fe_store(ta.out_ch, 0, v);
        }
    }
}

template <int K, int D, int EXTRA>
constexpr int pipe_block_threads() {
    return kPipeThreads;
}
// ... 431 lines not shown
```

zk_amd/csrc/round_kernels.cuh:

```cuda
#pragma once
#include "common.cuh"
#include "quad.cuh"

namespace zk {

template <int NS, bool SKIP1 = false>
ZK_D void block_reduce_store(Fe (&sum)[NS], uint64_t *__restrict__ partials, const FieldParams &P) {
    __shared__ uint32_t red[kBlock / 64][NS][8];
    const int lane = threadIdx.x & 63, wave = threadIdx.x >> 6;
#pragma unroll
    for (int t = 0; t < NS; ++t) {
        if (SKIP1 && t == 1) continue;
        sum[t] = fe_wave_sum(sum[t], P);
        if (lane == 0) {
#pragma unroll
            for (int i = 0; i < 8; ++i) red[wave][t][i] = sum[t].v[i];
        }
    }
    __syncthreads();
    if (threadIdx.x < NS && !(SKIP1 && threadIdx.x == 1)) {
        const int t = threadIdx.x;
        Fe acc;
#pragma unroll
        for (int i = 0; i < 8; ++i) acc.v[i] = red[0][t][i];
        for (int w = 1; w < kBlock / 64; ++w) {
            Fe o;
#pragma unroll
            for (int i = 0; i < 8; ++i) o.v[i] = red[w][t][i];
            acc = fe_add(acc, o, P);
        }
        fe_store(partials, (uint64_t)blockIdx.x * NS + t, acc);
    }
}

template <int D, bool FUSED>
__global__ __launch_bounds__(kBlock) void k_round(FactorPtrs fp, int k, uint64_t q, FieldParams P,
                                                  const uint64_t *__restrict__ rptr, uint64_t *__restrict__ partials) {
    constexpr int NS = D + 1;
    Mul29 r = {};
    if (FUSED) r = load_challenge29(rptr);
    Fe sum[NS];
    WideAcc acc[NS];
#pragma unroll
    for (int t = 0; t < NS; ++t) {
        sum[t] = fe_zero();
        wide_zero(acc[t]);
    }
    int lazy = 0;
    const uint64_t stride = (uint64_t)gridDim.x * kBlock;
    for (uint64_t j = (uint64_t)blockIdx.x * kBlock + threadIdx.x; j < q; j += stride) {
        Fe prod[NS];
        for (int f = 0; f < k; ++f) {
            Fe lo, hi;
            if (FUSED) {
                const Fe a0 = fe_load(fp.in[f], j), a1 = fe_load(fp.in[f], j + q);
                const Fe a2 = fe_load(fp.in[f], j + 2 * q), a3 = fe_load(fp.in[f], j + 3 * q);
                lo = fe_sub(a0, fe_mul29(fe_sub(a0, a2, P), r, P), P);
                hi = fe_sub(a1, fe_mul29(fe_sub(a1, a3, P), r, P), P);
                fe_store(fp.out[f], j, lo);
                fe_store(fp.out[f], j + q, hi);
            } else {
                lo = fe_load(fp.in[f], j);
                hi = fe_load(fp.in[f], j + q);
            }
            const Fe diff = fe_sub(hi, lo, P);
            Fe v = lo;
#pragma unroll
            for (int t = 0; t < NS; ++t) {
                if (t == 1) v = hi;
                else if (t > 1) v = fe_add(v, diff, P);
                if (k == 1) sum[t] = fe_add(sum[t], v, P);
                else if (f == 0) prod[t] = v;
                else if (f < k - 1) prod[t] = fe_mul(prod[t], v, P);
                else wide_mac(acc[t], prod[t].v, v.v);
            }
        }
        if (k > 1 && ++lazy == kMaxLazy) {
#pragma unroll
            for (int t = 0; t < NS; ++t) {
                sum[t] = fe_add(sum[t], redc_wide(acc[t], P), P);
                wide_zero(acc[t]);
            }
            lazy = 0;
        }
    }
    if (k > 1 && lazy) {
#pragma unroll
        for (int t = 0; t < NS; ++t) sum[t] = fe_add(sum[t], redc_wide(acc[t], P), P);
    }
    block_reduce_store<NS>(sum, partials, P);
}

#ifndef ZK_KD_INNER_MUL
#define ZK_KD_INNER_MUL fe_mul
#endif
template <int K, int D, bool FUSED, int EXTRA = 0>
struct RoundRegs {
    static constexpr int NS = D + 1, NL = FUSED ? 4 : 2;
    static constexpr bool DEEP = !FUSED && K + EXTRA <= 2;
    Fe cur[K + EXTRA][NL];
    Fe nxt[DEEP ? K + EXTRA : 1][DEEP ? NL : 1];
    Fe prod[NS];
    Fe sum[NS];
    Fe sum_b[EXTRA ? NS : 1];
    WideAcc acc[K > 1 ? NS : 1];
};
template <int F, int K, int D, bool FUSED, int EXTRA, bool SKIP1 = false, bool LEAD = false>
ZK_D void round_factor(RoundRegs<K, D, FUSED, EXTRA> &R, const FactorPtrs &fp, uint64_t j, uint64_t jn, bool more, uint64_t q,
                       const Mul29 &r, const FieldParams &P, uint64_t jnn = 0, bool more2 = false) {
    static_assert(!LEAD || (K == D && D >= 1), "the leading-coefficient slot needs deg = K = D");
    constexpr int NS = D + 1, NL = FUSED ? 4 : 2;
    constexpr bool PAIR3 = K == 3 && D == 3 && F == 1 && LEAD && !SKIP1;
    Fe lo, hi;
    if (FUSED) {
        lo = fe_sub(R.cur[F][0], fe_mul29(fe_sub(R.cur[F][0], R.cur[F][2], P), r, P), P);
        hi = fe_sub(R.cur[F][1], fe_mul29(fe_sub(R.cur[F][1], R.cur[F][3], P), r, P), P);
        fe_store(fp.out[F], j, lo);
        fe_store(fp.out[F], j + q, hi);
    } else {
        lo = R.cur[F][0];
        hi = R.cur[F][1];
    }
    constexpr bool DEEP = RoundRegs<K, D, FUSED, EXTRA>::DEEP;
    if (!DEEP) {
        if (more) {
#pragma unroll
            for (int l = 0; l < NL; ++l) R.cur[F][l] = fe_load(fp.in[F], jn + (uint64_t)l * q);
        }
    } else {
#pragma unroll
        for (int l = 0; l < NL; ++l) R.cur[F][l] = R.nxt[F][l];
        if (more2) {
#pragma unroll
            for (int l = 0; l < NL; ++l) R.nxt[F][l] = fe_load(fp.in[F], jnn + (uint64_t)l * q);
        }
    }
    const Fe diff = fe_sub(hi, lo, P);
    Fe v = lo;
#pragma unroll
    for (int t = 0; t < NS; ++t) {
        if (LEAD && t == D) v = diff;
        else if (t == 1) v = hi;
        else if (t > 1) v = fe_add(v, diff, P);
        if (SKIP1 && t == 1) continue;
        if (LEAD && t == D && F == K) continue;
        if (F == K) R.sum_b[t] = fe_add(R.sum_b[t], v, P);
        else if (K == 1) R.sum[t] = fe_add(R.sum[t], v, P);
        else if (F == 0) R.prod[t] = v;
        else if (PAIR3 && t == 2) continue;
        else if (F < K - 1) R.prod[t] = ZK_KD_INNER_MUL(R.prod[t], v, P);
        else wide_mac(R.acc[t], R.prod[t].v, v.v);
    }
    if (PAIR3) {
        const Fe bc = fe_add(R.prod[1], R.prod[3], P);
        R.prod[2] = fe_sub(fe_add(bc, bc, P), R.prod[0], P);
    }
}
#ifndef ZK_KD_MIN_BLOCKS
#define ZK_KD_MIN_BLOCKS(K, EXTRA, FUSED, SKIP1) (((K) + (EXTRA) <= 2 || ((K) == 3 && (EXTRA) == 0) || ((EXTRA) == 1 && (FUSED) && (SKIP1))) ? 2 : 1)
#endif
template <int K, int D, bool FUSED, int EXTRA = 0, bool SKIP1 = false, bool LEAD = false>
ZK_D void round_kd_body(const FactorPtrs &fp, uint64_t q, const FieldParams &P, const uint64_t *__restrict__ rptr, uint64_t *__restrict__ partials,
                        const ClaimJob &cj) {
    constexpr int NS = D + 1, NL = FUSED ? 4 : 2;
    uint32_t nblk = gridDim.x;
    if constexpr (SKIP1) {
        if (cj.out) {
            nblk -= 1;
            if (blockIdx.x == nblk) {
                if (threadIdx.x < 64) {
                    const Fe claim = claim_eval(cj, P);
                    if (threadIdx.x == 0) fe_store(cj.out, 0, claim);
                }
                return;
            }
        }
    }
    Mul29 r = {};
    if (FUSED) r = load_challenge29(rptr);
    RoundRegs<K, D, FUSED, EXTRA> R;
#pragma unroll
    for (int t = 0; t < NS; ++t) {
        R.sum[t] = fe_zero();
        if (EXTRA) R.sum_b[t] = fe_zero();
        if (K > 1) wide_zero(R.acc[t]);
    }
    const uint64_t stride = (uint64_t)nblk * kBlock;
    uint64_t j = (uint64_t)blockIdx.x * kBlock + threadIdx.x;
    if (j < q) {
#pragma unroll
        for (int f = 0; f < K + EXTRA; ++f)
#pragma unroll
            for (int l = 0; l < NL; ++l) R.cur[f][l] = fe_load(fp.in[f], j + (uint64_t)l * q);
    }
    if (RoundRegs<K, D, FUSED, EXTRA>::DEEP && j + stride < q) {
#pragma unroll
        for (int f = 0; f < K + EXTRA; ++f)
#pragma unroll
            for (int l = 0; l < NL; ++l) R.nxt[f][l] = fe_load(fp.in[f], j + stride + (uint64_t)l * q);
    }
    while (j < q) {
        const uint64_t jn = j + stride, jnn = jn + stride;
        const bool more = jn < q, more2 = jnn < q;
        round_factor<0, K, D, FUSED, EXTRA, SKIP1, LEAD>(R, fp, j, jn, more, q, r, P, jnn, more2);
        if constexpr (K + EXTRA > 1) round_factor<1, K, D, FUSED, EXTRA, SKIP1, LEAD>(R, fp, j, jn, more, q, r, P, jnn, more2);
        if constexpr (K + EXTRA > 2) round_factor<2, K, D, FUSED, EXTRA, SKIP1, LEAD>(R, fp, j, jn, more, q, r, P, jnn, more2);
        if constexpr (K + EXTRA > 3) round_factor<3, K, D, FUSED, EXTRA, SKIP1, LEAD>(R, fp, j, jn, more, q, r, P, jnn, more2);
        j = jn;
    }
    if (K > 1) {
#pragma unroll
        for (int t = 0; t < NS; ++t)
            if (!(SKIP1 && t == 1)) R.sum[t] = redc_wide(R.acc[t], P);
    }
    if (EXTRA) {
#pragma unroll
        for (int t = 0; t < NS; ++t)
            if (!(SKIP1 && t == 1)) R.sum[t] = fe_add(R.sum[t], R.sum_b[t], P);
    }
    block_reduce_store<NS, SKIP1>(R.sum, partials, P);
}
template <int K, int D, bool FUSED, int EXTRA = 0, bool SKIP1 = false, bool LEAD = false>
__global__ __launch_bounds__(kBlock, ZK_KD_MIN_BLOCKS(K, EXTRA, FUSED, SKIP1)) void k_round_kd(FactorPtrs fp, uint64_t q, FieldParams P,
                                                        const uint64_t *__restrict__ rptr, uint64_t *__restrict__ partials, ClaimJob cj = {}) {
    round_kd_body<K, D, FUSED, EXTRA, SKIP1, LEAD>(fp, q, P, rptr, partials, cj);
}
struct RoundSlot {
    FactorPtrs4 fp;
    const uint64_t *rptr;
    uint64_t *partials;
    ClaimJob cj;
};
template <int K, int D, bool FUSED, int EXTRA = 0, bool SKIP1 = false, bool LEAD = false>
__global__ __launch_bounds__(kBlock, ZK_KD_MIN_BLOCKS(K, EXTRA, FUSED, SKIP1)) void k_round_kd_b(BatchOf<RoundSlot> b, uint64_t q, FieldParams P) {
    const RoundSlot &a = b.a[blockIdx.y];
    const FactorPtrs fp = factor_ptrs_of(a.fp);
    round_kd_body<K, D, FUSED, EXTRA, SKIP1, LEAD>(fp, q, P, a.rptr, a.partials, a.cj);
}

ZK_D void dot29_mac(uint64_t (&c)[17], const uint32_t (&x)[9], const uint32_t (&y)[9]) {
#if defined(__HIP_DEVICE_COMPILE__) && !defined(ZK_NO_ASM)
    asm("v_mad_u64_u32 %0, vcc, %13, %18, %0\n\t"
        "v_mad_u64_u32 %1, vcc, %13, %19, %1\n\t"
        "v_mad_u64_u32 %2, vcc, %13, %20, %2\n\t"
        "v_mad_u64_u32 %3, vcc, %13, %21, %3\n\t"
        "v_mad_u64_u32 %4, vcc, %13, %22, %4\n\t"
        "v_mad_u64_u32 %5, vcc, %13, %23, %5\n\t"
        "v_mad_u64_u32 %6, vcc, %13, %24, %6\n\t"
        "v_mad_u64_u32 %7, vcc, %13, %25, %7\n\t"
        "v_mad_u64_u32 %8, vcc, %13, %26, %8\n\t"
        "v_mad_u64_u32 %1, vcc, %14, %18, %1\n\t"
        "v_mad_u64_u32 %2, vcc, %14, %19, %2\n\t"
        "v_mad_u64_u32 %3, vcc, %14, %20, %3\n\t"
        "v_mad_u64_u32 %4, vcc, %14, %21, %4\n\t"
        "v_mad_u64_u32 %5, vcc, %14, %22, %5\n\t"
        "v_mad_u64_u32 %6, vcc, %14, %23, %6\n\t"
        "v_mad_u64_u32 %7, vcc, %14, %24, %7\n\t"
        "v_mad_u64_u32 %8, vcc, %14, %25, %8\n\t"
        "v_mad_u64_u32 %9, vcc, %14, %26, %9\n\t"
        "v_mad_u64_u32 %2, vcc, %15, %18, %2\n\t"
        "v_mad_u64_u32 %3, vcc, %15, %19, %3\n\t"
        "v_mad_u64_u32 %4, vcc, %15, %20, %4\n\t"
        "v_mad_u64_u32 %5, vcc, %15, %21, %5\n\t"
        "v_mad_u64_u32 %6, vcc, %15, %22, %6\n\t"
        "v_mad_u64_u32 %7, vcc, %15, %23, %7\n\t"
        "v_mad_u64_u32 %8, vcc, %15, %24, %8\n\t"
        "v_mad_u64_u32 %9, vcc, %15, %25, %9\n\t"
        "v_mad_u64_u32 %10, vcc, %15, %26, %10\n\t"
        "v_mad_u64_u32 %3, vcc, %16, %18, %3\n\t"
        "v_mad_u64_u32 %4, vcc, %16, %19, %4\n\t"
        "v_mad_u64_u32 %5, vcc, %16, %20, %5\n\t"
        "v_mad_u64_u32 %6, vcc, %16, %21, %6\n\t"
        "v_mad_u64_u32 %7, vcc, %16, %22, %7\n\t"
        "v_mad_u64_u32 %8, vcc, %16, %23, %8\n\t"
        "v_mad_u64_u32 %9, vcc, %16, %24, %9\n\t"
        "v_mad_u64_u32 %10, vcc, %16, %25, %10\n\t"
        "v_mad_u64_u32 %11, vcc, %16, %26, %11\n\t"
        "v_mad_u64_u32 %4, vcc, %17, %18, %4\n\t"
        "v_mad_u64_u32 %5, vcc, %17, %19, %5\n\t"
        "v_mad_u64_u32 %6, vcc, %17, %20, %6\n\t"
        "v_mad_u64_u32 %7, vcc, %17, %21, %7\n\t"
        "v_mad_u64_u32 %8, vcc, %17, %22, %8\n\t"
        "v_mad_u64_u32 %9, vcc, %17, %23, %9\n\t"
        "v_mad_u64_u32 %10, vcc, %17, %24, %10\n\t"
        "v_mad_u64_u32 %11, vcc, %17, %25, %11\n\t"
        "v_mad_u64_u32 %12, vcc, %17, %26, %12"
        : "+v"(c[0]), "+v"(c[1]), "+v"(c[2]), "+v"(c[3]), "+v"(c[4]), "+v"(c[5]), "+v"(c[6]), "+v"(c[7]), "+v"(c[8]), "+v"(c[9]), "+v"(c[10]), "+v"(c[11]), "+v"(c[12])
        : "v"(x[0]), "v"(x[1]), "v"(x[2]), "v"(x[3]), "v"(x[4]), "v"(y[0]), "v"(y[1]), "v"(y[2]), "v"(y[3]), "v"(y[4]), "v"(y[5]), "v"(y[6]), "v"(y[7]), "v"(y[8])
        : "vcc");
    asm("v_mad_u64_u32 %0, vcc, %12, %16, %0\n\t"
        "v_mad_u64_u32 %1, vcc, %12, %17, %1\n\t"
        "v_mad_u64_u32 %2, vcc, %12, %18, %2\n\t"
        "v_mad_u64_u32 %3, vcc, %12, %19, %3\n\t"
        "v_mad_u64_u32 %4, vcc, %12, %20, %4\n\t"
        "v_mad_u64_u32 %5, vcc, %12, %21, %5\n\t"
        "v_mad_u64_u32 %6, vcc, %12, %22, %6\n\t"
        "v_mad_u64_u32 %7, vcc, %12, %23, %7\n\t"
        "v_mad_u64_u32 %8, vcc, %12, %24, %8\n\t"
        "v_mad_u64_u32 %1, vcc, %13, %16, %1\n\t"
        "v_mad_u64_u32 %2, vcc, %13, %17, %2\n\t"
        "v_mad_u64_u32 %3, vcc, %13, %18, %3\n\t"
        "v_mad_u64_u32 %4, vcc, %13, %19, %4\n\t"
        "v_mad_u64_u32 %5, vcc, %13, %20, %5\n\t"
        "v_mad_u64_u32 %6, vcc, %13, %21, %6\n\t"
        "v_mad_u64_u32 %7, vcc, %13, %22, %7\n\t"
        "v_mad_u64_u32 %8, vcc, %13, %23, %8\n\t"
        "v_mad_u64_u32 %9, vcc, %13, %24, %9\n\t"
        "v_mad_u64_u32 %2, vcc, %14, %16, %2\n\t"
        "v_mad_u64_u32 %3, vcc, %14, %17, %3\n\t"
        "v_mad_u64_u32 %4, vcc, %14, %18, %4\n\t"
        "v_mad_u64_u32 %5, vcc, %14, %19, %5\n\t"
        "v_mad_u64_u32 %6, vcc, %14, %20, %6\n\t"
        "v_mad_u64_u32 %7, vcc, %14, %21, %7\n\t"
        "v_mad_u64_u32 %8, vcc, %14, %22, %8\n\t"
        "v_mad_u64_u32 %9, vcc, %14, %23, %9\n\t"
        "v_mad_u64_u32 %10, vcc, %14, %24, %10\n\t"
        "v_mad_u64_u32 %3, vcc, %15, %16, %3\n\t"
        "v_mad_u64_u32 %4, vcc, %15, %17, %4\n\t"
        "v_mad_u64_u32 %5, vcc, %15, %18, %5\n\t"
        "v_mad_u64_u32 %6, vcc, %15, %19, %6\n\t"
        "v_mad_u64_u32 %7, vcc, %15, %20, %7\n\t"
        "v_mad_u64_u32 %8, vcc, %15, %21, %8\n\t"
        "v_mad_u64_u32 %9, vcc, %15, %22, %9\n\t"
        "v_mad_u64_u32 %10, vcc, %15, %23, %10\n\t"
        "v_mad_u64_u32 %11, vcc, %15, %24, %11"
        : "+v"(c[5]), "+v"(c[6]), "+v"(c[7]), "+v"(c[8]), "+v"(c[9]), "+v"(c[10]), "+v"(c[11]), "+v"(c[12]), "+v"(c[13]), "+v"(c[14]), "+v"(c[15]), "+v"(c[16])
        : "v"(x[5]), "v"(x[6]), "v"(x[7]), "v"(x[8]), "v"(y[0]), "v"(y[1]), "v"(y[2]), "v"(y[3]), "v"(y[4]), "v"(y[5]), "v"(y[6]), "v"(y[7]), "v"(y[8])
        : "vcc");
#else
#pragma unroll
    for (int i = 0; i < 9; ++i)
#pragma unroll
        for (int j = 0; j < 9; ++j) c[i + j] += (uint64_t)x[i] * y[j];
#endif
}

ZK_D void dot29_normalise(uint64_t (&c)[17]) {
    constexpr uint64_t M = (1ull << 29) - 1;
#pragma unroll
    for (int k = 0; k < 16; ++k) {
        c[k + 1] += c[k] >> 29;
        c[k] &= M;
    }
}
ZK_D void dot29_to_wide(const uint64_t (&c)[17], WideAcc &w) {
    constexpr uint64_t M = (1ull << 29) - 1;
    uint64_t window = 0;
    int have = 0, wi = 0;
#pragma unroll
    for (int k = 0; k < 18; ++k) {
        const uint64_t limb = k < 16 ? c[k] : (k == 16 ? (c[16] & M) : (c[16] >> 29));
        window |= limb << have;
        have += 29;
        if (have >= 32) {
            if (wi < 17) w.v[wi] = (uint32_t)window;
            ++wi;
            window >>= 32;
            have -= 32;
        }
    }
    if (wi < 17) w.v[wi++] = (uint32_t)window;
#pragma unroll
    for (int i = 0; i < 17; ++i)
        if (i >= wi) w.v[i] = 0;
}
template <int EXTRA>
ZK_D void round0_dot29_body(const FactorPtrs &fp, uint64_t q, const FieldParams &P, uint64_t *__restrict__ partials) {
    constexpr int NT = 2 + EXTRA;
    uint64_t c0[17], c1[17], cL[17];
#pragma unroll
    for (int k = 0; k < 17; ++k) c0[k] = c1[k] = cL[k] = 0;
    Fe sb0 = fe_zero(), sb1 = fe_zero();
    constexpr bool DEEP = EXTRA == 0;
    Fe cur[NT][2], nxt[DEEP ? NT : 1][2];
    const uint64_t stride = (uint64_t)gridDim.x * kBlock;
    uint64_t j = (uint64_t)blockIdx.x * kBlock + threadIdx.x;
    if (j < q) {
#pragma unroll
        for (int f = 0; f < NT; ++f) cur[f][0] = fe_load(fp.in[f], j), cur[f][1] = fe_load(fp.in[f], j + q);
    }
    if (DEEP && j + stride < q) {
#pragma unroll
        for (int f = 0; f < NT; ++f) nxt[f][0] = fe_load(fp.in[f], j + stride), nxt[f][1] = fe_load(fp.in[f], j + stride + q);
    }
    int since = 0;
    while (j < q) {
        const uint64_t jn = j + stride, jnn = jn + stride;
        Fe v[NT][2];
#pragma unroll
        for (int f = 0; f < NT; ++f) v[f][0] = cur[f][0], v[f][1] = cur[f][1];
        if (DEEP) {
#pragma unroll
            for (int f = 0; f < NT; ++f) cur[f][0] = nxt[f][0], cur[f][1] = nxt[f][1];
            if (jnn < q) {
#pragma unroll
                for (int f = 0; f < NT; ++f) nxt[f][0] = fe_load(fp.in[f], jnn), nxt[f][1] = fe_load(fp.in[f], jnn + q);
            }
        } else if (jn < q) {
#pragma unroll
            for (int f = 0; f < NT; ++f) cur[f][0] = fe_load(fp.in[f], jn), cur[f][1] = fe_load(fp.in[f], jn + q);
        }
        uint32_t a[9], b[9];
        split29(v[0][0].v, a);
        split29(v[1][0].v, b);
        dot29_mac(c0, a, b);
        split29(v[0][1].v, a);
        split29(v[1][1].v, b);
        dot29_mac(c1, a, b);
        const Fe d0 = fe_sub(v[0][1], v[0][0], P), d1 = fe_sub(v[1][1], v[1][0], P);
        split29(d0.v, a);
        split29(d1.v, b);
        dot29_mac(cL, a, b);
        if (EXTRA) {
            sb0 = fe_add(sb0, v[NT - 1][0], P);
            sb1 = fe_add(sb1, v[NT - 1][1], P);
        }
        if (++since == 7) {
            dot29_normalise(c0);
            dot29_normalise(c1);
            dot29_normalise(cL);
            since = 0;
        }
        j = jn;
    }
    dot29_normalise(c0);
    dot29_normalise(c1);
    dot29_normalise(cL);
    Fe sum[3];
    {
        WideAcc w;
        dot29_to_wide(c0, w);
        sum[0] = redc_wide(w, P);
        dot29_to_wide(c1, w);
        sum[1] = redc_wide(w, P);
        dot29_to_wide(cL, w);
        sum[2] = redc_wide(w, P);
    }
    if (EXTRA) {
        sum[0] = fe_add(sum[0], sb0, P);
        sum[1] = fe_add(sum[1], sb1, P);
    }
    block_reduce_store<3>(sum, partials, P);
}
template <int EXTRA>
__global__ __launch_bounds__(kBlock, 2) void k_round0_dot29(FactorPtrs fp, uint64_t q, FieldParams P, uint64_t *__restrict__ partials) {
    round0_dot29_body<EXTRA>(fp, q, P, partials);
}
template <int EXTRA>
__global__ __launch_bounds__(kBlock, 2) void k_round0_dot29_b(BatchOf<RoundSlot> b, uint64_t q, FieldParams P) {
    const RoundSlot &a = b.a[blockIdx.y];
    const FactorPtrs fp = factor_ptrs_of(a.fp);
    round0_dot29_body<EXTRA>(fp, q, P, a.partials);
}

extern __shared__ __attribute__((aligned(1024))) uint8_t glds_ring[];
constexpr uint32_t kGldsRingBytes = 4 * 8192, kGldsRing3Bytes = 4 * 12288;
template <int N>
ZK_D void wait_vm() {
    asm volatile("s_waitcnt vmcnt(%0)" ::"n"(N) : "memory");
}
#define ZK_GLDS_PIECES(ADDR)                      \
    "global_load_lds_dwordx4 %1, " ADDR " nt\n\t" \
    "global_load_lds_dwordx4 %1, " ADDR " offset:1024 nt\n\t"
#define ZK_GLDS_ROW(M0, ADDR) "s_mov_b32 m0, " M0 "\n\ts_nop 0\n\t" ZK_GLDS_PIECES(ADDR)
ZK_D void glds_rows2(uint64_t a0, uint64_t a1, uint32_t voff, uint32_t lds_dst) {
    unsigned keep;
    asm volatile("s_mov_b32 %0, m0\n\t" ZK_GLDS_ROW("%4", "%2") ZK_GLDS_ROW("%5", "%3") "s_mov_b32 m0, %0"
                 : "=&s"(keep)
                 : "v"(voff), "s"(a0), "s"(a1), "s"(lds_dst), "s"(lds_dst + 2048u)
                 : "memory");
}
ZK_D void glds_rows4(uint64_t a0, uint64_t a1, uint64_t a2, uint64_t a3, uint32_t voff, uint32_t lds_dst) {
    unsigned keep;
    asm volatile("s_mov_b32 %0, m0\n\t" ZK_GLDS_ROW("%6", "%2") ZK_GLDS_ROW("%7", "%3") ZK_GLDS_ROW("%8", "%4") ZK_GLDS_ROW("%9", "%5") "s_mov_b32 m0, %0"
                 : "=&s"(keep)
                 : "v"(voff), "s"(a0), "s"(a1), "s"(a2), "s"(a3), "s"(lds_dst), "s"(lds_dst + 2048u), "s"(lds_dst + 4096u), "s"(lds_dst + 6144u)
                 : "memory");
}
#undef ZK_GLDS_ROW
#undef ZK_GLDS_PIECES
ZK_D Fe glds_elem(const uint8_t *row, uint32_t elem) {
    const uint4 *p = reinterpret_cast<const uint4 *>(row + elem * 32);
    const uint4 a = p[0], b = p[1];
    Fe r = {{a.x, a.y, a.z, a.w, b.x, b.y, b.z, b.w}};
    return r;
}
struct GldsWave {
    uint8_t *my;
    uint32_t my_lds;
    uint32_t lane, voff, own;
    uint64_t r0, rs, K;
};
ZK_D GldsWave glds_wave(uint64_t q, uint32_t nblk, uint32_t bytes_per_wave = 8192) {
    GldsWave w;
    w.lane = threadIdx.x & 63;
    const uint32_t wave = __builtin_amdgcn_readfirstlane(threadIdx.x >> 6);
    w.my = glds_ring + wave * bytes_per_wave;
    w.my_lds = __builtin_amdgcn_readfirstlane((uint32_t)(uintptr_t)w.my);
    w.voff = w.lane * 16;
    w.own = pair_owned(w.lane);
    const uint64_t runs = q >> 6;
    w.r0 = (uint64_t)blockIdx.x * (kBlock / 64) + wave;
    w.rs = (uint64_t)nblk * (kBlock / 64);
    w.K = w.r0 < runs ? (runs - w.r0 + w.rs - 1) / w.rs : 0;
    return w;
}

template <int NU, int F>
ZK_D void round0_glds_wait(bool last) {
    if (!last) wait_vm<4 * (NU - 1)>();
    else wait_vm<4 * (NU - 1 - F)>();
}
ZK_D void dot29_flush(uint64_t (&c)[17], Fe &sum, const FieldParams &P) {
    WideAcc wa;
    dot29_to_wide(c, wa);
    sum = fe_add(sum, redc_wide(wa, P), P);
#pragma unroll
    for (int i = 0; i < 17; ++i) c[i] = 0;
}
template <int EXTRA>
ZK_D void round0_glds_body(const FactorPtrs &fp, uint64_t q, const FieldParams &P, uint64_t *__restrict__ partials) {
    constexpr int NU = 2 + EXTRA;
    const GldsWave w = glds_wave(q, gridDim.x, NU * 4096);
    const uint64_t hi_off = q * 32;
    uint64_t c0[17], c1[17], cL[17];
#pragma unroll
    for (int k = 0; k < 17; ++k) c0[k] = c1[k] = cL[k] = 0;
    Fe sum[3] = {fe_zero(), fe_zero(), fe_zero()};
    Fe sb0 = fe_zero(), sb1 = fe_zero();
    if (w.K) {
#pragma unroll
        for (int f = 0; f < NU; ++f) {
            const uint64_t a = (uint64_t)(uintptr_t)fp.in[f] + w.r0 * 2048;
            glds_rows2(a, a + hi_off, w.voff, w.my_lds + f * 4096);
        }
        int since = 0, lazy = 0;
        for (uint64_t k = 0; k < w.K; ++k) {
            const bool last = k + 1 == w.K;
            const uint64_t next = (w.r0 + (k + 1) * w.rs) * 2048;
            uint32_t la0[9], la1[9], ld0[9];
            round0_glds_wait<NU, 0>(last);
            {
                const Fe lo = glds_elem(w.my, w.lane), hi = glds_elem(w.my + 2048, w.lane);
                asm volatile("s_waitcnt lgkmcnt(0)" ::: "memory");
                if (!last) glds_rows2((uint64_t)(uintptr_t)fp.in[0] + next, (uint64_t)(uintptr_t)fp.in[0] + next + hi_off, w.voff, w.my_lds);
                split29(lo.v, la0);
                split29(hi.v, la1);
                const Fe d = fe_sub(hi, lo, P);
                split29(d.v, ld0);
            }
            round0_glds_wait<NU, 1>(last);
            {
                const Fe lo = glds_elem(w.my + 4096, w.lane), hi = glds_elem(w.my + 6144, w.lane);
                asm volatile("s_waitcnt lgkmcnt(0)" ::: "memory");
                if (!last) glds_rows2((uint64_t)(uintptr_t)fp.in[1] + next, (uint64_t)(uintptr_t)fp.in[1] + next + hi_off, w.voff, w.my_lds + 4096);
                uint32_t b[9];
                split29(lo.v, b);
                dot29_mac(c0, la0, b);
                split29(hi.v, b);
                dot29_mac(c1, la1, b);
                const Fe d = fe_sub(hi, lo, P);
                split29(d.v, b);
                dot29_mac(cL, ld0, b);
            }
            if constexpr (EXTRA) {
                round0_glds_wait<NU, 2>(last);
                const Fe lo = glds_elem(w.my + 8192, w.lane), hi = glds_elem(w.my + 10240, w.lane);
                asm volatile("s_waitcnt lgkmcnt(0)" ::: "memory");
                if (!last) glds_rows2((uint64_t)(uintptr_t)fp.in[2] + next, (uint64_t)(uintptr_t)fp.in[2] + next + hi_off, w.voff, w.my_lds + 8192);
                sb0 = fe_add(sb0, lo, P);
                sb1 = fe_add(sb1, hi, P);
            }
            ++lazy;
            if (++since == 7 || lazy == kMaxLazy || last) {
                dot29_normalise(c0);
                dot29_normalise(c1);
                dot29_normalise(cL);
                since = 0;
            }
            if (lazy == kMaxLazy || last) {
                dot29_flush(c0, sum[0], P);
                dot29_flush(c1, sum[1], P);
                dot29_flush(cL, sum[2], P);
                lazy = 0;
            }
        }
    }
    if (EXTRA) {
        sum[0] = fe_add(sum[0], sb0, P);
        sum[1] = fe_add(sum[1], sb1, P);
    }
    block_reduce_store<3>(sum, partials, P);
}
template <int EXTRA>
__global__ __launch_bounds__(kBlock, 2) void k_round0_glds(FactorPtrs fp, uint64_t q, FieldParams P, uint64_t *__restrict__ partials) {
    round0_glds_body<EXTRA>(fp, q, P, partials);
}
template <int EXTRA>
__global__ __launch_bounds__(kBlock, 2) void k_round0_glds_b(BatchOf<RoundSlot> b, uint64_t q, FieldParams P) {
    const RoundSlot &a = b.a[blockIdx.y];
    const FactorPtrs fp = factor_ptrs_of(a.fp);
    round0_glds_body<EXTRA>(fp, q, P, a.partials);
}

template <int F, int K, int EXTRA, bool STORE_NT>
ZK_D void fused_glds_unit(const GldsWave &w, const FactorPtrs &fp, uint64_t q, uint64_t run, bool last, const Mul29 &r, const FieldParams &P,
                          Fe (&prod)[K + 1], WideAcc (&acc)[K + 1], Fe (&sum_b)[K + 1]) {
    constexpr int D = K, NT = K + EXTRA;
    const Fe c0 = glds_elem(w.my, w.own), c1 = glds_elem(w.my + 2048, w.own), c2 = glds_elem(w.my + 4096, w.own), c3 = glds_elem(w.my + 6144, w.own);
    asm volatile("s_waitcnt lgkmcnt(0)" ::: "memory");
    const uint64_t rowb = q * 32;
    if (F + 1 < NT) {
        const uint64_t a = (uint64_t)(uintptr_t)fp.in[F + 1 < NT ? F + 1 : 0] + run * 2048;
        glds_rows4(a, a + rowb, a + 2 * rowb, a + 3 * rowb, w.voff, w.my_lds);
    } else if (!last) {
        const uint64_t a = (uint64_t)(uintptr_t)fp.in[0] + (run + w.rs) * 2048;
        glds_rows4(a, a + rowb, a + 2 * rowb, a + 3 * rowb, w.voff, w.my_lds);
    }
    const Fe lo = fe_sub(c0, fe_mul29(fe_sub(c0, c2, P), r, P), P);
    const Fe hi = fe_sub(c1, fe_mul29(fe_sub(c1, c3, P), r, P), P);
    uint64_t *out = fp.out[F];
    if (STORE_NT) {
        run_store_nt(out + run * 256, w.lane, lo);
        run_store_nt(out + (run * 64 + q) * 4, w.lane, hi);
    } else {
        run_store(out + run * 256, w.lane, lo);
        run_store(out + (run * 64 + q) * 4, w.lane, hi);
    }
    const Fe diff = fe_sub(hi, lo, P);
    Fe v = lo;
#pragma unroll
    for (int t = 0; t <= D; ++t) {
        if (t == 1) {
            v = hi;
            continue;
        }
        if (t == D) v = diff;
        else if (t > 1) v = fe_add(v, diff, P);
        if (F == K) {
            if (t < D) sum_b[t] = fe_add(sum_b[t], v, P);
        } else if (F == 0) prod[t] = v;
        else if (F < K - 1) prod[t] = ZK_KD_INNER_MUL(prod[t], v, P);
        else wide_mac(acc[t], prod[t].v, v.v);
    }
    if (F + 1 < NT || !last) wait_vm<4>();
}
template <int K, int EXTRA, bool STORE_NT>
ZK_D void fused_glds_body(const FactorPtrs &fp, uint64_t q, const FieldParams &P, const uint64_t *__restrict__ rptr, uint64_t *__restrict__ partials,
                          const ClaimJob &cj) {
    constexpr int NS = K + 1;
    uint32_t nblk = gridDim.x;
    if (cj.out) {
        nblk -= 1;
        if (blockIdx.x == nblk) {
            if (threadIdx.x < 64) {
                const Fe claim = claim_eval(cj, P);
                if (threadIdx.x == 0) fe_store(cj.out, 0, claim);
            }
            return;
        }
    }
    const Mul29 r = load_challenge29(rptr);
    asm volatile("s_waitcnt vmcnt(0)" ::: "memory");
    const GldsWave w = glds_wave(q, nblk);
    Fe prod[NS], sum[NS], sum_b[NS];
    WideAcc acc[NS];
#pragma unroll
    for (int t = 0; t < NS; ++t) {
        sum[t] = fe_zero();
        sum_b[t] = fe_zero();
        wide_zero(acc[t]);
    }
    if (w.K) {
        {
            const uint64_t a = (uint64_t)(uintptr_t)fp.in[0] + w.r0 * 2048, rowb = q * 32;
            glds_rows4(a, a + rowb, a + 2 * rowb, a + 3 * rowb, w.voff, w.my_lds);
        }
        wait_vm<0>();
        for (uint64_t k = 0; k < w.K; ++k) {
            const uint64_t run = w.r0 + k * w.rs;
            const bool last = k + 1 == w.K;
            fused_glds_unit<0, K, EXTRA, STORE_NT>(w, fp, q, run, last, r, P, prod, acc, sum_b);
            fused_glds_unit<1, K, EXTRA, STORE_NT>(w, fp, q, run, last, r, P, prod, acc, sum_b);
            if constexpr (K + EXTRA > 2) fused_glds_unit<2, K, EXTRA, STORE_NT>(w, fp, q, run, last, r, P, prod, acc, sum_b);
            if constexpr (K + EXTRA > 3) fused_glds_unit<3, K, EXTRA, STORE_NT>(w, fp, q, run, last, r, P, prod, acc, sum_b);
        }
#pragma unroll
        for (int t = 0; t < NS; ++t)
            if (t != 1) sum[t] = redc_wide(acc[t], P);
        if (EXTRA) {
#pragma unroll
            for (int t = 0; t < K; ++t)
                if (t != 1) sum[t] = fe_add(sum[t], sum_b[t], P);
        }
    }
    block_reduce_store<NS, true>(sum, partials, P);
}
template <int K, int EXTRA, bool STORE_NT>
__global__ __launch_bounds__(kBlock, 2) void k_round_fused_glds(FactorPtrs fp, uint64_t q, FieldParams P, const uint64_t *__restrict__ rptr,
                                                                 uint64_t *__restrict__ partials, ClaimJob cj) {
    fused_glds_body<K, EXTRA, STORE_NT>(fp, q, P, rptr, partials, cj);
}
template <int K, int EXTRA, bool STORE_NT>
__global__ __launch_bounds__(kBlock, 2) void k_round_fused_glds_b(BatchOf<RoundSlot> b, uint64_t q, FieldParams P) {
    const RoundSlot &a = b.a[blockIdx.y];
    const FactorPtrs fp = factor_ptrs_of(a.fp);
    fused_glds_body<K, EXTRA, STORE_NT>(fp, q, P, a.rptr, a.partials, a.cj);
}

template <int K, int D, int EXTRA>
ZK_D void round_quad_body(const FactorPtrs &fp, uint64_t q, const FieldParams &P, const uint64_t *__restrict__ rptr, uint64_t *__restrict__ partials) {
    constexpr int NF = K + EXTRA, NS = D + 1;
    static_assert(NF <= 4 && NS <= 4, "four lanes per pair index");
    __shared__ uint32_t red[kBlock / 64][4][8];
    const Mul29 r = load_challenge29(rptr);
    const uint32_t lane = threadIdx.x & 63, wave = threadIdx.x >> 6, l4 = lane & 3;
    const bool has_factor = l4 < (uint32_t)NF;
    const uint64_t *in = fp.in[0];
    uint64_t *out = fp.out[0];
#pragma unroll
    for (int f = 1; f < NF; ++f)
        if (l4 == (uint32_t)f) {
            in = fp.in[f];
            out = fp.out[f];
        }
    const uint64_t stride = (uint64_t)gridDim.x * (kBlock / 4);
    uint64_t j = (uint64_t)blockIdx.x * (kBlock / 4) + (threadIdx.x >> 2);
    WideAcc acc;
    wide_zero(acc);
    Fe sum = fe_zero();
    Fe cur[4];
#pragma unroll
    for (int l = 0; l < 4; ++l) cur[l] = fe_zero();
    if (j < q && has_factor) {
#pragma unroll
        for (int l = 0; l < 4; ++l) cur[l] = fe_load(in, j + (uint64_t)l * q);
    }
    while (j < q) {
        const uint64_t jn = j + stride;
        Fe v[NS];
        v[0] = fe_sub(cur[0], fe_mul29(fe_sub(cur[0], cur[2], P), r, P), P);
        const Fe hi = fe_sub(cur[1], fe_mul29(fe_sub(cur[1], cur[3], P), r, P), P);
        if (has_factor) {
            fe_store(out, j, v[0]);
            fe_store(out, j + q, hi);
            if (jn < q) {
#pragma unroll
                for (int l = 0; l < 4; ++l) cur[l] = fe_load(in, jn + (uint64_t)l * q);
            }
        }
        if constexpr (NS > 1) v[1] = hi;
        if constexpr (NS > 2) {
            const Fe diff = fe_sub(hi, v[0], P);
#pragma unroll
            for (int t = 2; t < NS; ++t) v[t] = fe_add(v[t - 1], diff, P);
        }
        Fe w[NF];
#pragma unroll
        for (int g = 0; g < NF; ++g) w[g] = fe_zero();
        quad_transpose<0, NF, NS>(v, w, l4);
        if constexpr (K == 1) {
            sum = fe_add(sum, w[0], P);
        } else {
            Fe prod = w[0];
#pragma unroll
            for (int g = 1; g + 1 < K; ++g) prod = ZK_KD_INNER_MUL(prod, w[g], P);
            wide_mac(acc, prod.v, w[K - 1].v);
        }
        if constexpr (EXTRA) sum = fe_add(sum, w[K], P);
        j = jn;
    }
    Fe s = sum;
    if constexpr (K > 1) s = fe_add(redc_wide(acc, P), sum, P);
    {
        Fe a, b;
#pragma unroll
        for (int i = 0; i < 8; ++i) {
            const auto x = __builtin_amdgcn_permlane32_swap(s.v[i], s.v[i], false, false);
            a.v[i] = x[0];
            b.v[i] = x[1];
        }
        s = fe_add(a, b, P);
#pragma unroll
        for (int i = 0; i < 8; ++i) {
            const auto x = __builtin_amdgcn_permlane16_swap(s.v[i], s.v[i], false, false);
            a.v[i] = x[0];
            b.v[i] = x[1];
        }
        s = fe_add(a, b, P);
        s = fe_add(s, fe_dpp<0x128>(s), P);
        s = fe_add(s, fe_dpp<0x12C>(s), P);
    }
    if (lane < 4) {
#pragma unroll
        for (int i = 0; i < 8; ++i) red[wave][lane][i] = s.v[i];
    }
    __syncthreads();
    if (threadIdx.x < (uint32_t)NS) {
        Fe tot = fe_zero();
        for (int wv = 0; wv < kBlock / 64; ++wv) {
            Fe o;
#pragma unroll
            for (int i = 0; i < 8; ++i) o.v[i] = red[wv][threadIdx.x][i];
            tot = fe_add(tot, o, P);
        }
        fe_store(partials, (uint64_t)blockIdx.x * NS + threadIdx.x, tot);
    }
}
template <int K, int D, int EXTRA>
__global__ __launch_bounds__(kBlock) void k_round_quad(FactorPtrs fp, uint64_t q, FieldParams P, const uint64_t *__restrict__ rptr,
                                                       uint64_t *__restrict__ partials) {
    round_quad_body<K, D, EXTRA>(fp, q, P, rptr, partials);
}
template <int K, int D, int EXTRA>
__global__ __launch_bounds__(kBlock) void k_round_quad_b(BatchOf<RoundSlot> b, uint64_t q, FieldParams P) {
    const RoundSlot &a = b.a[blockIdx.y];
    const FactorPtrs fp = factor_ptrs_of(a.fp);
    round_quad_body<K, D, EXTRA>(fp, q, P, a.rptr, a.partials);
}

__global__ __launch_bounds__(kBlock) void k_round_single_t(FactorPtrs fp, int k, uint64_t q, FieldParams P, Fe tval,
                                                           uint64_t *__restrict__ partials) {
    Fe sum[1] = {fe_zero()};
    const uint64_t stride = (uint64_t)gridDim.x * kBlock;
    for (uint64_t j = (uint64_t)blockIdx.x * kBlock + threadIdx.x; j < q; j += stride) {
        Fe prod = fe_zero();
        for (int f = 0; f < k; ++f) {
            const Fe lo = fe_load(fp.in[f], j), hi = fe_load(fp.in[f], j + q);
            const Fe v = fe_sub(lo, fe_mul(tval, fe_sub(lo, hi, P), P), P);
            prod = (f == 0) ? v : fe_mul(prod, v, P);
        }
        sum[0] = fe_add(sum[0], prod, P);
    }
    block_reduce_store<1>(sum, partials, P);
}

}
```

zk_amd/csrc/rounds.hip:

```cpp
#include <cstdlib>

#include "env.hpp"
#include "launch.hpp"
#include "round_kernels.cuh"

namespace zk {

static constexpr uint32_t kCapGrid = 2048;

static uint32_t min_blocks() {
    static const uint32_t v = (uint32_t)env_u64("ZK_ROUND_MIN_BLOCKS", 512, 1, 2048);
    return v;
}
static int round0_dot29_mode() {
    static const int v = (int)env_u64("ZK_ROUND0_DOT29", 1, 0, 2);
    return v;
}
static bool round0_dot29() { return round0_dot29_mode() != 0; }
static bool round0_dot29_extra() { return round0_dot29_mode() == 2; }
static bool glds_rounds() {
    static const bool v = env_u64("ZK_ROUND_GLDS", 1, 0, 1) != 0;
    return v;
}
static uint64_t glds_min_pairs(uint64_t unset) {
    static const uint64_t v = env_u64("ZK_ROUND_GLDS_MIN_PAIRS", 0, 0, (uint64_t)1 << 40);
    return v ? v : unset;
}
static uint64_t glds_nt_min_pairs() {
    static const uint64_t v = env_u64("ZK_ROUND_GLDS_NT_MIN_PAIRS", (uint64_t)1 << 20, 64, (uint64_t)1 << 40);
    return v;
}
static bool glds_takes(uint64_t q, uint64_t min_pairs) { return glds_rounds() && (q & 63) == 0 && q >= 64 && q >= glds_min_pairs(min_pairs); }
static uint64_t quad_max_pairs() {
    static const uint64_t v = env_u64("ZK_QUAD_MAX_PAIRS", (uint64_t)1 << 15, 0, (uint64_t)1 << 40);
    return v;
}
template <int K, int D, int EXTRA>
static uint32_t launch_quad(const RoundLaunchCtx &lc, const FactorPtrs &fp, uint64_t q, const uint64_t *d_r) {
    uint64_t g = (q + 63) / 64;
    const uint64_t cap = (q + 64ull * kMaxLazy - 1) / (64ull * kMaxLazy);
    if (g > 2048) g = cap > 2048 ? cap : 2048;
    const FieldParams *P = lc.P;
    hipStream_t st = lc.stream;
    uint64_t *part = lc.d_partials;
    const uint32_t grid = (uint32_t)g;
    auto single = [=]() {
        k_round_quad<K, D, EXTRA><<<grid, kBlock, 0, st>>>(fp, q, *P, d_r, part);
        return hipGetLastError();
    };
    if (!batch_record(BK_ROUND_QUAD, (uint32_t)K | ((uint32_t)D << 4) | ((uint32_t)EXTRA << 9), grid, kBlock, 0, q, 0, 0, 0,
                      RoundSlot{factor_ptrs4(fp), d_r, part, ClaimJob{}}, single))
        (void)single();
    return grid;
}
static uint32_t min_blocks_plus1() {
    static const uint32_t v = (uint32_t)env_u64("ZK_ROUND_MIN_BLOCKS", 256, 1, 2048);
    return v;
}
static inline uint32_t round_grid(uint64_t q, uint32_t min_b = min_blocks()) {
    uint64_t b = (q + (uint64_t)kBlock * kMaxLazy - 1) / ((uint64_t)kBlock * kMaxLazy);
    const uint64_t one_pair = (q + kBlock - 1) / kBlock;
    const uint64_t floor_b = one_pair < min_b ? one_pair : min_b;
    if (b < floor_b) b = floor_b;
    return (uint32_t)(b ? b : 1);
}
static inline uint32_t capped_grid(uint64_t q) {
    uint64_t b = (q + kBlock - 1) / kBlock;
    if (b > kCapGrid) b = kCapGrid;
    return (uint32_t)(b ? b : 1);
}

static inline uint32_t claim_blocks(const RoundLaunchCtx &lc) { return lc.claim.out ? 1u : 0u; }

thread_local BatchRecorder *g_batch = nullptr;

constexpr uint32_t kd_shape(int K, int D, bool FUSED, int EXTRA, bool SKIP1, bool LEAD) {
    return (uint32_t)K | ((uint32_t)D << 4) | ((uint32_t)FUSED << 8) | ((uint32_t)EXTRA << 9) | ((uint32_t)SKIP1 << 10) | ((uint32_t)LEAD << 11);
}
template <int K, int D, bool FUSED, int EXTRA = 0, bool SKIP1 = false, bool LEAD = false>
static void go_kd(const RoundLaunchCtx &lc, const FactorPtrs &fp, uint64_t q, const uint64_t *d_r, uint32_t grid, const ClaimJob &cj = {}) {
    const FieldParams *P = lc.P;
    hipStream_t st = lc.stream;
    uint64_t *part = lc.d_partials;
    auto single = [=]() {
        k_round_kd<K, D, FUSED, EXTRA, SKIP1, LEAD><<<grid, kBlock, 0, st>>>(fp, q, *P, d_r, part, cj);
        return hipGetLastError();
    };
    if (batch_record(BK_ROUND_KD, kd_shape(K, D, FUSED, EXTRA, SKIP1, LEAD), grid, kBlock, 0, q, 0, 0, 0, RoundSlot{factor_ptrs4(fp), d_r, part, cj}, single))
        return;
    (void)single();
}
template <int EXTRA>
static void go_round0_dot29(const RoundLaunchCtx &lc, const FactorPtrs &fp, uint64_t q, uint32_t grid) {
    const FieldParams *P = lc.P;
    hipStream_t st = lc.stream;
    uint64_t *part = lc.d_partials;
    auto single = [=]() {
        k_round0_dot29<EXTRA><<<grid, kBlock, 0, st>>>(fp, q, *P, part);
        return hipGetLastError();
    };
    if (batch_record(BK_ROUND0_DOT29, (uint32_t)EXTRA, grid, kBlock, 0, q, 0, 0, 0, RoundSlot{factor_ptrs4(fp), nullptr, part, ClaimJob{}}, single)) return;
    (void)single();
}

constexpr uint32_t kShapeGlds = 1u << 12, kShapeGldsNt = 1u << 13;
template <int EXTRA>
static void go_round0_glds(const RoundLaunchCtx &lc, const FactorPtrs &fp, uint64_t q, uint32_t grid) {
    const FieldParams *P = lc.P;
    hipStream_t st = lc.stream;
    uint64_t *part = lc.d_partials;
    constexpr uint32_t lds = EXTRA ? kGldsRing3Bytes : kGldsRingBytes;
    auto single = [=]() {
        k_round0_glds<EXTRA><<<grid, kBlock, lds, st>>>(fp, q, *P, part);
        return hipGetLastError();
    };
    if (batch_record(BK_ROUND0_DOT29, kShapeGlds | (uint32_t)EXTRA, grid, kBlock, lds, q, 0, 0, 0, RoundSlot{factor_ptrs4(fp), nullptr, part, ClaimJob{}}, single)) return;
    (void)single();
}
template <int K, int EXTRA>
static void go_fused_glds(const RoundLaunchCtx &lc, const FactorPtrs &fp, uint64_t q, const uint64_t *d_r, uint32_t grid, const ClaimJob &cj) {
    const FieldParams *P = lc.P;
    hipStream_t st = lc.stream;
    uint64_t *part = lc.d_partials;
    const bool nt = q >= glds_nt_min_pairs();
    auto single = [=]() {
        if (nt) k_round_fused_glds<K, EXTRA, true><<<grid, kBlock, kGldsRingBytes, st>>>(fp, q, *P, d_r, part, cj);
        else k_round_fused_glds<K, EXTRA, false><<<grid, kBlock, kGldsRingBytes, st>>>(fp, q, *P, d_r, part, cj);
        return hipGetLastError();
    };
    if (batch_record(BK_ROUND_KD, kd_shape(K, K, true, EXTRA, true, true) | kShapeGlds | (nt ? kShapeGldsNt : 0u), grid, kBlock, kGldsRingBytes, q, 0, 0, 0,
                     RoundSlot{factor_ptrs4(fp), d_r, part, cj}, single))
        return;
    (void)single();
}

template <int K, int D>
static void launch_kd(const RoundLaunchCtx &lc, const FactorPtrs &fp, uint64_t q, bool fused, const uint64_t *d_r, uint32_t g) {
    if (fused) go_kd<K, D, true>(lc, fp, q, d_r, g);
    else go_kd<K, D, false>(lc, fp, q, d_r, g);
}
template <int D>
static void launch_generic(const RoundLaunchCtx &lc, const FactorPtrs &fp, int k, uint64_t q, bool fused, const uint64_t *d_r, uint32_t g) {
    const FieldParams *P = lc.P;
    hipStream_t st = lc.stream;
    uint64_t *part = lc.d_partials;
    auto single = [=]() {
        if (fused) k_round<D, true><<<g, kBlock, 0, st>>>(fp, k, q, *P, d_r, part);
        else k_round<D, false><<<g, kBlock, 0, st>>>(fp, k, q, *P, d_r, part);
        return hipGetLastError();
    };
    if (!batch_record_other(single)) (void)single();
}

int launch_round(const RoundLaunchCtx &lc, const FactorPtrs &fp, int k, uint64_t q, uint32_t D, bool fused,
                 const uint64_t *d_r, uint32_t *out_grid, bool *skip1, bool *lead) {
    if (D < 1 || D > 4 || k < 1 || k > kMaxFactors) return kLaunchUnsupported;
    uint32_t g = round_grid(q);
    bool no_lead = false;
    if (!lead) lead = &no_lead;
    if (*lead && !((k == 2 && D == 2) || (k == 3 && D == 3))) *lead = false;
    if (*lead && (uint64_t)g * (D + 1) <= lc.capacity_elems) {
        const int shl = k * 10 + (int)D;
        bool done = true;
        if (!fused) {
            if (shl == 22 && round0_dot29() && glds_takes(q, (uint64_t)1 << 21)) {
                if (g > 512) g = 512;
                go_round0_glds<0>(lc, fp, q, g);
            } else if (shl == 22 && round0_dot29()) go_round0_dot29<0>(lc, fp, q, g);
            else if (shl == 22) go_kd<2, 2, false, 0, false, true>(lc, fp, q, d_r, g);
            else go_kd<3, 3, false, 0, false, true>(lc, fp, q, d_r, g);
            if (skip1) *skip1 = false;
        } else if (skip1 && *skip1) {
            if (shl == 33 && glds_takes(q, (uint64_t)1 << 16)) go_fused_glds<3, 0>(lc, fp, q, d_r, g + claim_blocks(lc), lc.claim);
            else if (shl == 22) go_kd<2, 2, true, 0, true, true>(lc, fp, q, d_r, g + claim_blocks(lc), lc.claim);
            else go_kd<3, 3, true, 0, true, true>(lc, fp, q, d_r, g + claim_blocks(lc), lc.claim);
        } else {
            done = false;
        }
        if (done) {
            if (hipGetLastError() != hipSuccess) return kLaunchHipError;
            *out_grid = g;
            return kLaunchOk;
        }
    }
    *lead = false;
    if (fused && q >= 16 && q <= 4 * quad_max_pairs() && (uint64_t)2048 * (D + 1) <= lc.capacity_elems) {
        const int shq = k * 10 + (int)D;
        uint32_t gq = 0;
        if (shq == 22 && q <= quad_max_pairs()) gq = launch_quad<2, 2, 0>(lc, fp, q, d_r);
        else if (shq == 33) gq = launch_quad<3, 3, 0>(lc, fp, q, d_r);
        if (gq) {
            if (skip1) *skip1 = false;
            if (hipGetLastError() != hipSuccess) return kLaunchHipError;
            *out_grid = gq;
            return kLaunchOk;
        }
    }
    if (skip1 && *skip1) {
        const bool fits1 = (uint64_t)g * (D + 1) <= lc.capacity_elems;
        const int shape1 = (fits1 && fused) ? k * 10 + (int)D : 0;
        if (shape1 == 22) go_kd<2, 2, true, 0, true>(lc, fp, q, d_r, g + claim_blocks(lc), lc.claim);
        else if (shape1 == 33) go_kd<3, 3, true, 0, true>(lc, fp, q, d_r, g + claim_blocks(lc), lc.claim);
        else *skip1 = false;
        if (*skip1) {
            if (hipGetLastError() != hipSuccess) return kLaunchHipError;
            *out_grid = g;
            return kLaunchOk;
        }
    }
    const bool fits = (uint64_t)g * (D + 1) <= lc.capacity_elems;
    const int shape = fits ? k * 10 + (int)D : 0;
    switch (shape) {
        case 11: launch_kd<1, 1>(lc, fp, q, fused, d_r, g); break;
        case 12: launch_kd<1, 2>(lc, fp, q, fused, d_r, g); break;
        case 21: launch_kd<2, 1>(lc, fp, q, fused, d_r, g); break;
        case 22: launch_kd<2, 2>(lc, fp, q, fused, d_r, g); break;
        case 23: launch_kd<2, 3>(lc, fp, q, fused, d_r, g); break;
        case 32: launch_kd<3, 2>(lc, fp, q, fused, d_r, g); break;
        case 33: launch_kd<3, 3>(lc, fp, q, fused, d_r, g); break;
        default:
            g = capped_grid(q);
            switch (D) {
                case 1: launch_generic<1>(lc, fp, k, q, fused, d_r, g); break;
                case 2: launch_generic<2>(lc, fp, k, q, fused, d_r, g); break;
                case 3: launch_generic<3>(lc, fp, k, q, fused, d_r, g); break;
                default: launch_generic<4>(lc, fp, k, q, fused, d_r, g); break;
            }
    }
    if (hipGetLastError() != hipSuccess) return kLaunchHipError;
    *out_grid = g;
    return kLaunchOk;
}

int launch_round_plus1(const RoundLaunchCtx &lc, const FactorPtrs &fp, int k, uint64_t q, uint32_t D, bool fused,
                       const uint64_t *d_r, uint32_t *out_grid, bool *skip1, bool *lead) {
    uint32_t g = round_grid(q, min_blocks_plus1());
    if ((uint64_t)g * (D + 1) > lc.capacity_elems) return kLaunchUnsupported;
    const int shape = k * 10 + (int)D;
    bool no_lead = false;
    if (!lead) lead = &no_lead;
    if (*lead && shape == 22 && (!fused || (skip1 && *skip1))) {
        if (!fused) {
            if (round0_dot29_extra()) go_round0_dot29<1>(lc, fp, q, g);
            else if (round0_dot29() && glds_takes(q, (uint64_t)1 << 20)) {
                if (g > 512) g = 512;
                go_round0_glds<1>(lc, fp, q, g);
            } else go_kd<2, 2, false, 1, false, true>(lc, fp, q, d_r, g);
            if (skip1) *skip1 = false;
        } else {
            if (glds_takes(q, (uint64_t)1 << 19)) go_fused_glds<2, 1>(lc, fp, q, d_r, g + claim_blocks(lc), lc.claim);
            else go_kd<2, 2, true, 1, true, true>(lc, fp, q, d_r, g + claim_blocks(lc), lc.claim);
        }
        if (hipGetLastError() != hipSuccess) return kLaunchHipError;
        *out_grid = g;
        return kLaunchOk;
    }
    *lead = false;
    if (fused && shape == 22 && q >= 16 && q <= quad_max_pairs() && (uint64_t)2048 * (D + 1) <= lc.capacity_elems) {
        const uint32_t gq = launch_quad<2, 2, 1>(lc, fp, q, d_r);
        if (skip1) *skip1 = false;
        if (hipGetLastError() != hipSuccess) return kLaunchHipError;
        *out_grid = gq;
        return kLaunchOk;
    }
    if (skip1 && *skip1 && !(shape == 22 && fused)) *skip1 = false;
    if (shape == 22) {
        if (fused && skip1 && *skip1) go_kd<2, 2, true, 1, true>(lc, fp, q, d_r, g + claim_blocks(lc), lc.claim);
        else if (fused) go_kd<2, 2, true, 1>(lc, fp, q, d_r, g);
        else go_kd<2, 2, false, 1>(lc, fp, q, d_r, g);
    } else if (shape == 33) {
        if (fused) go_kd<3, 3, true, 1>(lc, fp, q, d_r, g);
        else go_kd<3, 3, false, 1>(lc, fp, q, d_r, g);
    } else {
        return kLaunchUnsupported;
    }
    if (hipGetLastError() != hipSuccess) return kLaunchHipError;
    *out_grid = g;
    return kLaunchOk;
}

int launch_round_single_t(const RoundLaunchCtx &lc, const FactorPtrs &fp, int k, uint64_t q, const Fe &tval, uint32_t *out_grid) {
    const uint32_t g = capped_grid(q);
    {
        const FieldParams *P = lc.P;
        hipStream_t st = lc.stream;
        uint64_t *part = lc.d_partials;
        auto single = [=]() {
            k_round_single_t<<<g, kBlock, 0, st>>>(fp, k, q, *P, tval, part);
            return hipGetLastError();
        };
        if (!batch_record_other(single)) (void)single();
    }
    if (hipGetLastError() != hipSuccess) return kLaunchHipError;
    *out_grid = g;
    return kLaunchOk;
}

int batch_launch_rounds(const BatchRecorder &r, size_t idx) {
    const BatchRecord &r0 = r.recs[0][idx];
    BatchOf<RoundSlot> slots;
    batch_gather(r, idx, slots);
    const dim3 grid(r0.grid, (uint32_t)r.n);
    const uint64_t q = r0.s[0];
    const FieldParams &P = *r.P;
#define ZK_KD_B(K, D, F, E, S, L)                                                                  \
    case kd_shape(K, D, F, E, S, L):                                                               \
        k_round_kd_b<K, D, F, E, S, L><<<grid, kBlock, 0, r.stream>>>(slots, q, P);               \
        break;
    if (r0.kernel == BK_ROUND_KD && (r0.shape & kShapeGlds)) {
        const uint32_t base = r0.shape & ~(kShapeGlds | kShapeGldsNt);
        const bool nt = (r0.shape & kShapeGldsNt) != 0;
        if (base == kd_shape(3, 3, true, 0, true, true)) {
            if (nt) k_round_fused_glds_b<3, 0, true><<<grid, kBlock, kGldsRingBytes, r.stream>>>(slots, q, P);
            else k_round_fused_glds_b<3, 0, false><<<grid, kBlock, kGldsRingBytes, r.stream>>>(slots, q, P);
        } else {
            return kLaunchUnsupported;
        }
    } else if (r0.kernel == BK_ROUND_KD) {
        switch (r0.shape) {
            ZK_KD_B(2, 2, true, 0, true, true)
            ZK_KD_B(3, 3, true, 0, true, true)
            ZK_KD_B(3, 3, false, 0, false, true)
            ZK_KD_B(2, 2, true, 0, false, false)
            ZK_KD_B(3, 3, true, 0, false, false)
            ZK_KD_B(2, 2, false, 0, false, false)
            ZK_KD_B(3, 3, false, 0, false, false)
            default: return kLaunchUnsupported;
        }
// ... 20 lines not shown
```

Before: 195.7 billion.

## Store unreduced wide-accumulator partials and defer Montgomery reduction to tail kernels

Round kernels with K>1 now write per-block partial sums as 17-limb unreduced wide accumulators (9 u64 words) instead of reducing to field elements first. The tail kernels sum these wide records with carry-chain adds, using permlane swaps and DPP for the cross-lane reduction, and perform a single reduction at the end. This removes the per-block Montgomery reductions and modular adds, at the cost of larger partial records, more memory traffic in the tail, and a new overflow guard in the field setup. The round-0 GLDS grid sizing also changes so the grid can grow beyond 512 blocks when q is large.

After: 195.5 billion. About the same (-0.1%).

```diff
diff --git a/zk_amd/csrc/capi.hip b/zk_amd/csrc/capi.hip
--- a/zk_amd/csrc/capi.hip
+++ b/zk_amd/csrc/capi.hip
@@ -183,7 +183,7 @@
     HIPCHK(hipSetDevice(c->device));
     HIPCHK(hipStreamCreateWithFlags(&c->own_stream, hipStreamNonBlocking));
     c->stream = c->own_stream;
-    HIPCHK(hipMalloc(&c->d_partials, (size_t)kMaxGrid * kMaxSums * 32));
+    HIPCHK(hipMalloc(&c->d_partials, (size_t)kMaxGrid * kMaxSums * kWideRecWords * 8));
     HIPCHK(hipMalloc(&c->d_sums, (size_t)kMaxSums * 32 * 3));
     HIPCHK(hipHostMalloc(&c->h_pinned, (size_t)kMaxSums * 32 * 3, kPolledHostFlags));
     HIPCHK(hipHostMalloc((void **)&c->h_flag, 64 * kMaxBatch, kPolledHostFlags));
@@ -997,7 +997,9 @@
 }
 
 static inline uint64_t partials_capacity() { return g_batch ? (uint64_t)kMaxGrid * kMaxSums / kMaxBatch : (uint64_t)kMaxGrid * kMaxSums; }
-static inline uint64_t *partials_of(zk_ctx *c) { return g_batch ? c->d_partials + (size_t)g_batch->cur * partials_capacity() * 4 : c->d_partials; }
+static inline uint64_t *partials_of(zk_ctx *c) {
+    return g_batch ? c->d_partials + (size_t)g_batch->cur * partials_capacity() * kWideRecWords : c->d_partials;
+}
 static inline RoundLaunchCtx launch_ctx(zk_ctx *c) {
     RoundLaunchCtx lc = {c->stream, &c->fi->P, partials_of(c), partials_capacity(), {}};
     return lc;
@@ -1078,6 +1080,7 @@
     uint32_t blocks;
     bool skip1;
     bool lead;
+    bool wide;
     const uint64_t *claim;
 };
 static uint64_t lead_min_pairs() {
@@ -1098,6 +1101,7 @@
         const bool may_derive = !tt.lanes || (tt.lanes_dv && shard_skip_on());
         bool skip1 = dv && dv->prev_rp && tt.claim_park && fused && may_derive && D <= (uint32_t)kMaxSkipDegree && q >= skip1_min_pairs();
         bool lead = may_derive && q >= lead_min_pairs();
+        bool wide = false;
         ClaimJob cjob = {};
         if (skip1 && claim_in_round()) cjob = ClaimJob{dv->prev_rp, dv->prev_chal, dv->w, tt.claim_park, D + 1};
         auto with_claim = [&](RoundLaunchCtx lc) {
@@ -1107,6 +1111,7 @@
         auto tail_dv = [&]() {
             TailDerive t = skip1 && dv ? *dv : TailDerive{};
             t.lead = lead ? D : 0;
+            t.wide = wide ? 1 : 0;
             t.claim = (t.prev_rp && cjob.out) ? cjob.out : nullptr;
             if (tt.lanes) {
                 if (tt.lanes_dv) *tt.lanes_dv = t;
@@ -1117,7 +1122,7 @@
         if (tt.lanes_dv) *tt.lanes_dv = TailDerive{};
         if (ts.n_terms == 2 && ts.term_k[1] == 1) {
             uint32_t g = 0;
-            const int lrc = launch_round_plus1(with_claim(launch_ctx(c)), fp, ts.term_k[0], q, D, fused, d_r, &g, &skip1, &lead);
+            const int lrc = launch_round_plus1(with_claim(launch_ctx(c)), fp, ts.term_k[0], q, D, fused, d_r, &g, &skip1, &lead, &wide);
             if (lrc == kLaunchHipError) {
                 g_hip_err = "round kernel launch failed";
                 return ZK_ERR_HIP;
@@ -1128,6 +1133,7 @@
                     defer->skip1 = skip1;
                     defer->claim = skip1 ? cjob.out : nullptr;
                     defer->lead = lead;
+                    defer->wide = wide;
                     return ZK_OK;
                 }
                 return launch_tail(c, g, D + 1, tt.sponge, tt.out_rp, tt.out_ch, tt.d_challenge, tt.lanes, tail_dv(), tt.init);
@@ -1144,10 +1150,11 @@
                 sub.out[f] = fp.out[first + f];
             }
             RoundLaunchCtx lc = with_claim(launch_ctx(c));
-            lc.d_partials += (size_t)total * (D + 1) * 4;
+            wide = ts.n_terms != 1;
+            lc.d_partials += (size_t)total * (D + 1) * kWideRecWords;
             lc.capacity_elems -= (uint64_t)total * (D + 1);
             uint32_t g = 0;
-            const int lrc = launch_round(lc, sub, ts.term_k[i], q, D, fused, d_r, &g, &skip1, &lead);
+            const int lrc = launch_round(lc, sub, ts.term_k[i], q, D, fused, d_r, &g, &skip1, &lead, &wide);
             if (lrc == kLaunchUnsupported) return ZK_ERR_UNSUPPORTED;
             if (lrc != kLaunchOk) {
                 g_hip_err = "round kernel launch failed";
@@ -1161,6 +1168,7 @@
             defer->skip1 = skip1;
             defer->claim = skip1 ? cjob.out : nullptr;
             defer->lead = lead;
+            defer->wide = wide;
             return ZK_OK;
         }
         return launch_tail(c, total, D + 1, tt.sponge, tt.out_rp, tt.out_ch, tt.d_challenge, tt.lanes, tail_dv(), tt.init);
@@ -1552,6 +1560,7 @@
         pl.tail.dv.claim = dt.claim;
     }
     pl.tail.dv.lead = dt.lead ? st.D : 0;
+    pl.tail.dv.wide = dt.wide ? 1 : 0;
     FactorPtrs fp = {};
     for (uint64_t i = 0; i < st.k; ++i) fp.in[i] = fp.out[i] = st.cur[i];
     uint32_t g = 0;
@@ -1695,7 +1704,7 @@
         return finish_enqueue(st);
     }
     const uint64_t m_s = st.pending_fold ? st.vars_left - 1 : st.vars_left;
-    DeferredTail dt = {0, false, false, nullptr};
+    DeferredTail dt = {0, false, false, false, nullptr};
     const bool enter = fast_degree(st.D) && pipe_wants_next(st, m_s);
     ZKCHK(round_enqueue(st, nullptr, enter ? &dt : nullptr));
     if (enter && dt.blocks) ZKCHK(pipe_enter(st, dt));
diff --git a/zk_amd/csrc/common.cuh b/zk_amd/csrc/common.cuh
--- a/zk_amd/csrc/common.cuh
+++ b/zk_amd/csrc/common.cuh
@@ -117,6 +117,7 @@
     uint32_t local_only;
     const uint64_t *claim;
     uint32_t log_world;
+    uint32_t wide;
 };
 struct ClaimJob {
     const uint64_t *prev_rp;
@@ -170,6 +171,60 @@
     if (width > 2) s = fe_add(s, fe_dpp<0x12E>(s), P);
     if (width > 1) s = fe_add(s, fe_dpp<0x12F>(s), P);
     return s;
+}
+template <bool KEEP_QUADS = false>
+ZK_D void wide_wave_sum(WideAcc &s) {
+    WideAcc o;
+#pragma unroll
+    for (int i = 0; i < 17; ++i) {
+        const auto r = __builtin_amdgcn_permlane32_swap(s.v[i], s.v[i], false, false);
+        s.v[i] = r[0];
+        o.v[i] = r[1];
+    }
+    wide_add(s, o);
+#pragma unroll
+    for (int i = 0; i < 17; ++i) {
+        const auto r = __builtin_amdgcn_permlane16_swap(s.v[i], s.v[i], false, false);
+        s.v[i] = r[0];
+        o.v[i] = r[1];
+    }
+    wide_add(s, o);
+#pragma unroll
+    for (int i = 0; i < 17; ++i) o.v[i] = __builtin_amdgcn_update_dpp(0u, s.v[i], 0x128, 0xF, 0xF, true);
+    wide_add(s, o);
+#pragma unroll
+    for (int i = 0; i < 17; ++i) o.v[i] = __builtin_amdgcn_update_dpp(0u, s.v[i], 0x12C, 0xF, 0xF, true);
+    wide_add(s, o);
+    if (!KEEP_QUADS) {
+#pragma unroll
+        for (int i = 0; i < 17; ++i) o.v[i] = __builtin_amdgcn_update_dpp(0u, s.v[i], 0x12E, 0xF, 0xF, true);
+        wide_add(s, o);
+#pragma unroll
+        for (int i = 0; i < 17; ++i) o.v[i] = __builtin_amdgcn_update_dpp(0u, s.v[i], 0x12F, 0xF, 0xF, true);
+        wide_add(s, o);
+    }
+}
+#ifndef ZK_TAIL_WIDE_INFLIGHT
+#define ZK_TAIL_WIDE_INFLIGHT 8
+#endif
+constexpr int kTailWideInFlight = ZK_TAIL_WIDE_INFLIGHT;
+ZK_D void wide_store(uint64_t *base, uint64_t idx, const WideAcc &w) {
+    uint2 *p = reinterpret_cast<uint2 *>(base + idx * kWideRecWords);
+#pragma unroll
+    for (int i = 0; i < 8; ++i) p[i] = make_uint2(w.v[2 * i], w.v[2 * i + 1]);
+    p[8] = make_uint2(w.v[16], 0u);
+}
+ZK_D WideAcc wide_load(const uint64_t *base, uint64_t idx) {
+    const uint2 *p = reinterpret_cast<const uint2 *>(base + idx * kWideRecWords);
+    WideAcc w;
+#pragma unroll
+    for (int i = 0; i < 8; ++i) {
+        const uint2 x = p[i];
+        w.v[2 * i] = x.x;
+        w.v[2 * i + 1] = x.y;
+    }
+    w.v[16] = p[8].x;
+    return w;
 }
 ZK_D Fe claim_eval(const ClaimJob &cj, const FieldParams &P) {
     const uint32_t lane = threadIdx.x & 63;
diff --git a/zk_amd/csrc/field.cuh b/zk_amd/csrc/field.cuh
--- a/zk_amd/csrc/field.cuh
+++ b/zk_amd/csrc/field.cuh
@@ -381,6 +381,45 @@
     return r;
 }
 
+constexpr int kWideRecWords = 9;
+ZK_HD void wide_add(WideAcc &a, const WideAcc &b) {
+    uint32_t c = 0;
+#pragma unroll
+    for (int i = 0; i < 17; ++i) {
+        uint32_t co;
+        a.v[i] = __builtin_addc(a.v[i], b.v[i], c, &co);
+        c = co;
+    }
+}
+ZK_HD void wide_add_fe_hi(WideAcc &a, const Fe &s) {
+    uint32_t c = 0;
+#pragma unroll
+    for (int i = 8; i < 17; ++i) {
+        uint32_t co;
+        a.v[i] = __builtin_addc(a.v[i], i < 16 ? s.v[i - 8] : 0u, c, &co);
+        c = co;
+    }
+}
+ZK_HD Fe redc_wide_any(const WideAcc &w, const FieldParams &P) {
+    WideAcc f;
+    const uint32_t top = w.v[16];
+    uint64_t c = 0;
+#pragma unroll
+    for (int i = 0; i < 8; ++i) {
+        c += (uint64_t)top * P.r2[i] + w.v[i];
+        f.v[i] = (uint32_t)c;
+        c >>= 32;
+    }
+#pragma unroll
+    for (int i = 8; i < 16; ++i) {
+        c += w.v[i];
+        f.v[i] = (uint32_t)c;
+        c >>= 32;
+    }
+    f.v[16] = (uint32_t)c;
+    return redc_wide(f, P);
+}
+
 ZK_HD Fe fe_reduce_u256(const uint32_t x[8], const FieldParams &P) {
     uint32_t s[9];
 #pragma unroll
diff --git a/zk_amd/csrc/host_field.hpp b/zk_amd/csrc/host_field.hpp
--- a/zk_amd/csrc/host_field.hpp
+++ b/zk_amd/csrc/host_field.hpp
@@ -102,6 +102,7 @@
         const uint64_t rp = rp_log >= 0 && rp_log < 32 ? (1ull << rp_log) : ~0ull;
         const uint64_t top = top_log < 0 ? 0 : (top_log < 32 ? (1ull << top_log) : ~0ull);
         if (rp_log < 0 || rp + 1 + top >= 32 || rp + 1 + top < rp) return nullptr;
+        if (rp + 1 + 1 >= 32) return nullptr;
     }
     I.two_adicity = adicity[field];
     I.generator = gen[field];
diff --git a/zk_amd/csrc/kernels.cuh b/zk_amd/csrc/kernels.cuh
--- a/zk_amd/csrc/kernels.cuh
+++ b/zk_amd/csrc/kernels.cuh
@@ -362,6 +362,23 @@
             }
             term = fe_wave_sum(term, P, 8);
             if (lane == 0) claim = term;
+            continue;
+        }
+        if (dv.wide) {
+            WideAcc a;
+            wide_zero(a);
+            for (uint32_t b = lane; b < nblocks; b += kTailWideInFlight * 64) {
+                WideAcc x[kTailWideInFlight];
+#pragma unroll
+                for (int u = 0; u < kTailWideInFlight; ++u) {
+                    if (b + u * 64 < nblocks) x[u] = wide_load(partials, (uint64_t)(b + u * 64) * ns + t);
+                    else wide_zero(x[u]);
+                }
+#pragma unroll
+                for (int u = 0; u < kTailWideInFlight; ++u) wide_add(a, x[u]);
+            }
+            wide_wave_sum(a);
+            if (lane == 0) fin[t] = redc_wide_any(a, P);
             continue;
         }
         Fe s = fe_zero();
diff --git a/zk_amd/csrc/launch.hpp b/zk_amd/csrc/launch.hpp
--- a/zk_amd/csrc/launch.hpp
+++ b/zk_amd/csrc/launch.hpp
@@ -73,9 +73,9 @@
 };
 enum { kLaunchOk = 0, kLaunchUnsupported = -1, kLaunchHipError = -2 };
 int launch_round(const RoundLaunchCtx &lc, const FactorPtrs &fp, int k, uint64_t q, uint32_t D, bool fused,
-                 const uint64_t *d_r, uint32_t *out_grid, bool *skip1 = nullptr, bool *lead = nullptr);
+                 const uint64_t *d_r, uint32_t *out_grid, bool *skip1 = nullptr, bool *lead = nullptr, bool *wide = nullptr);
 int launch_round_plus1(const RoundLaunchCtx &lc, const FactorPtrs &fp, int k, uint64_t q, uint32_t D, bool fused,
-                       const uint64_t *d_r, uint32_t *out_grid, bool *skip1 = nullptr, bool *lead = nullptr);
+                       const uint64_t *d_r, uint32_t *out_grid, bool *skip1 = nullptr, bool *lead = nullptr, bool *wide = nullptr);
 int launch_round_single_t(const RoundLaunchCtx &lc, const FactorPtrs &fp, int k, uint64_t q, const Fe &tval, uint32_t *out_grid);
 
 
diff --git a/zk_amd/csrc/pipe_kernels.cuh b/zk_amd/csrc/pipe_kernels.cuh
--- a/zk_amd/csrc/pipe_kernels.cuh
+++ b/zk_amd/csrc/pipe_kernels.cuh
@@ -296,7 +296,26 @@
     if (wave0) dbg_stamp(ta.dbg, 0);
     if (wave0) sp = lane_sponge_load(ta.sponge, L);
     const uint32_t wave = __builtin_amdgcn_readfirstlane(tid >> 6);
-    if (ta.nblocks == 1) {
+    if (ta.mode == 0 && ta.dv.wide) {
+        if (wave < ta.n_in && !(wave == 1 && ta.dv.prev_rp)) {
+            WideAcc a;
+            wide_zero(a);
+            for (uint32_t b = lane; b < ta.nblocks; b += kTailWideInFlight * 64) {
+                WideAcc x[kTailWideInFlight];
+#pragma unroll
+                for (int u = 0; u < kTailWideInFlight; ++u) {
+                    if (b + u * 64 < ta.nblocks) x[u] = wide_load(ta.partials, (uint64_t)(b + u * 64) * ta.n_in + wave);
+                    else wide_zero(x[u]);
+                }
+#pragma unroll
+                for (int u = 0; u < kTailWideInFlight; ++u) wide_add(a, x[u]);
+            }
+            wide_wave_sum(a);
+            if (lane == 0) red[wave] = redc_wide_any(a, P);
+        }
+        __syncthreads();
+        if (wave >= 2) return;
+    } else if (ta.nblocks == 1) {
         if (wave >= 2) return;
         if (wave0 && lane < 16 && lane < ta.n_in) red[lane] = fe_load(ta.partials, lane);
     } else {
diff --git a/zk_amd/csrc/round_kernels.cuh b/zk_amd/csrc/round_kernels.cuh
--- a/zk_amd/csrc/round_kernels.cuh
+++ b/zk_amd/csrc/round_kernels.cuh
@@ -5,7 +5,7 @@
 namespace zk {
 
 template <int NS, bool SKIP1 = false>
-ZK_D void block_reduce_store(Fe (&sum)[NS], uint64_t *__restrict__ partials, const FieldParams &P) {
+ZK_D void block_reduce_store(Fe (&sum)[NS], uint64_t *__restrict__ partials, const FieldParams &P, uint32_t wide_rec = 0) {
     __shared__ uint32_t red[kBlock / 64][NS][8];
     const int lane = threadIdx.x & 63, wave = threadIdx.x >> 6;
 #pragma unroll
@@ -29,13 +29,48 @@
             for (int i = 0; i < 8; ++i) o.v[i] = red[w][t][i];
             acc = fe_add(acc, o, P);
         }
-        fe_store(partials, (uint64_t)blockIdx.x * NS + t, acc);
+        if (wide_rec) {
+            WideAcc w;
+            wide_zero(w);
+            wide_add_fe_hi(w, acc);
+            wide_store(partials, (uint64_t)blockIdx.x * NS + t, w);
+        } else {
+            fe_store(partials, (uint64_t)blockIdx.x * NS + t, acc);
+        }
+    }
+}
+template <int NS, bool SKIP1 = false>
+ZK_D void block_reduce_store_wide(WideAcc (&acc)[NS], uint64_t *__restrict__ partials) {
+    __shared__ uint32_t redw[kBlock / 64][NS][17];
+    const int lane = threadIdx.x & 63, wave = threadIdx.x >> 6;
+#pragma unroll
+    for (int t = 0; t < NS; ++t) {
+        if (SKIP1 && t == 1) continue;
+        wide_wave_sum(acc[t]);
+        if (lane == 0) {
+#pragma unroll
+            for (int i = 0; i < 17; ++i) redw[wave][t][i] = acc[t].v[i];
+        }
+    }
+    __syncthreads();
+    if (threadIdx.x < NS && !(SKIP1 && threadIdx.x == 1)) {
+        const int t = threadIdx.x;
+        WideAcc tot;
+#pragma unroll
+        for (int i = 0; i < 17; ++i) tot.v[i] = redw[0][t][i];
+        for (int w = 1; w < kBlock / 64; ++w) {
+            WideAcc o;
+#pragma unroll
+            for (int i = 0; i < 17; ++i) o.v[i] = redw[w][t][i];
+            wide_add(tot, o);
+        }
+        wide_store(partials, (uint64_t)blockIdx.x * NS + t, tot);
     }
 }
 
 template <int D, bool FUSED>
 __global__ __launch_bounds__(kBlock) void k_round(FactorPtrs fp, int k, uint64_t q, FieldParams P,
-                                                  const uint64_t *__restrict__ rptr, uint64_t *__restrict__ partials) {
+                                                  const uint64_t *__restrict__ rptr, uint64_t *__restrict__ partials, uint32_t wide_rec = 0) {
     constexpr int NS = D + 1;
     Mul29 r = {};
     if (FUSED) r = load_challenge29(rptr);
@@ -88,7 +123,7 @@
 #pragma unroll
         for (int t = 0; t < NS; ++t) sum[t] = fe_add(sum[t], redc_wide(acc[t], P), P);
     }
-    block_reduce_store<NS>(sum, partials, P);
+    block_reduce_store<NS>(sum, partials, P, wide_rec);
 }
 
 #ifndef ZK_KD_INNER_MUL
@@ -161,7 +196,7 @@
 #endif
 template <int K, int D, bool FUSED, int EXTRA = 0, bool SKIP1 = false, bool LEAD = false>
 ZK_D void round_kd_body(const FactorPtrs &fp, uint64_t q, const FieldParams &P, const uint64_t *__restrict__ rptr, uint64_t *__restrict__ partials,
-                        const ClaimJob &cj) {
+                        const ClaimJob &cj, uint32_t wide_rec = 0) {
     constexpr int NS = D + 1, NL = FUSED ? 4 : 2;
     uint32_t nblk = gridDim.x;
     if constexpr (SKIP1) {
@@ -208,22 +243,27 @@
         if constexpr (K + EXTRA > 3) round_factor<3, K, D, FUSED, EXTRA, SKIP1, LEAD>(R, fp, j, jn, more, q, r, P, jnn, more2);
         j = jn;
     }
-    if (K > 1) {
-#pragma unroll
-        for (int t = 0; t < NS; ++t)
-            if (!(SKIP1 && t == 1)) R.sum[t] = redc_wide(R.acc[t], P);
-    }
-    if (EXTRA) {
-#pragma unroll
-        for (int t = 0; t < NS; ++t)
-            if (!(SKIP1 && t == 1)) R.sum[t] = fe_add(R.sum[t], R.sum_b[t], P);
-    }
-    block_reduce_store<NS, SKIP1>(R.sum, partials, P);
+    if constexpr (K > 1) {
+        if (EXTRA) {
+#pragma unroll
+            for (int t = 0; t < NS; ++t)
+                if (!(SKIP1 && t == 1) && !(LEAD && t == D)) wide_add_fe_hi(R.acc[t], R.sum_b[t]);
+        }
+        block_reduce_store_wide<NS, SKIP1>(R.acc, partials);
+    } else {
+        if (EXTRA) {
+#pragma unroll
+            for (int t = 0; t < NS; ++t)
+                if (!(SKIP1 && t == 1)) R.sum[t] = fe_add(R.sum[t], R.sum_b[t], P);
+        }
+        block_reduce_store<NS, SKIP1>(R.sum, partials, P, wide_rec);
+    }
 }
 template <int K, int D, bool FUSED, int EXTRA = 0, bool SKIP1 = false, bool LEAD = false>
 __global__ __launch_bounds__(kBlock, ZK_KD_MIN_BLOCKS(K, EXTRA, FUSED, SKIP1)) void k_round_kd(FactorPtrs fp, uint64_t q, FieldParams P,
-                                                        const uint64_t *__restrict__ rptr, uint64_t *__restrict__ partials, ClaimJob cj = {}) {
-    round_kd_body<K, D, FUSED, EXTRA, SKIP1, LEAD>(fp, q, P, rptr, partials, cj);
+                                                        const uint64_t *__restrict__ rptr, uint64_t *__restrict__ partials, ClaimJob cj = {},
+                                                        uint32_t wide_rec = 0) {
+    round_kd_body<K, D, FUSED, EXTRA, SKIP1, LEAD>(fp, q, P, rptr, partials, cj, wide_rec);
 }
 struct RoundSlot {
     FactorPtrs4 fp;
@@ -365,6 +405,19 @@
         if (i >= wi) w.v[i] = 0;
 }
 template <int EXTRA>
+ZK_D void dot29_block_store(const uint64_t (&c0)[17], const uint64_t (&c1)[17], const uint64_t (&cL)[17], const Fe &sb0, const Fe &sb1,
+                            uint64_t *__restrict__ partials) {
+    WideAcc acc[3];
+    dot29_to_wide(c0, acc[0]);
+    dot29_to_wide(c1, acc[1]);
+    dot29_to_wide(cL, acc[2]);
+    if (EXTRA) {
+        wide_add_fe_hi(acc[0], sb0);
+        wide_add_fe_hi(acc[1], sb1);
+    }
+    block_reduce_store_wide<3>(acc, partials);
+}
+template <int EXTRA>
 ZK_D void round0_dot29_body(const FactorPtrs &fp, uint64_t q, const FieldParams &P, uint64_t *__restrict__ partials) {
     constexpr int NT = 2 + EXTRA;
     uint64_t c0[17], c1[17], cL[17];
@@ -426,21 +479,7 @@
     dot29_normalise(c0);
     dot29_normalise(c1);
     dot29_normalise(cL);
-    Fe sum[3];
-    {
-        WideAcc w;
-        dot29_to_wide(c0, w);
-        sum[0] = redc_wide(w, P);
-        dot29_to_wide(c1, w);
-        sum[1] = redc_wide(w, P);
-        dot29_to_wide(cL, w);
-        sum[2] = redc_wide(w, P);
-    }
-    if (EXTRA) {
-        sum[0] = fe_add(sum[0], sb0, P);
-        sum[1] = fe_add(sum[1], sb1, P);
-    }
-    block_reduce_store<3>(sum, partials, P);
+    dot29_block_store<EXTRA>(c0, c1, cL, sb0, sb1, partials);
 }
 template <int EXTRA>
 __global__ __launch_bounds__(kBlock, 2) void k_round0_dot29(FactorPtrs fp, uint64_t q, FieldParams P, uint64_t *__restrict__ partials) {
@@ -511,13 +550,7 @@
     if (!last) wait_vm<4 * (NU - 1)>();
     else wait_vm<4 * (NU - 1 - F)>();
 }
-ZK_D void dot29_flush(uint64_t (&c)[17], Fe &sum, const FieldParams &P) {
-    WideAcc wa;
-    dot29_to_wide(c, wa);
-    sum = fe_add(sum, redc_wide(wa, P), P);
-#pragma unroll
-    for (int i = 0; i < 17; ++i) c[i] = 0;
-}
+constexpr uint32_t kGldsRound0MaxRuns = 128;
 template <int EXTRA>
 ZK_D void round0_glds_body(const FactorPtrs &fp, uint64_t q, const FieldParams &P, uint64_t *__restrict__ partials) {
     constexpr int NU = 2 + EXTRA;
@@ -526,7 +559,6 @@
     uint64_t c0[17], c1[17], cL[17];
 #pragma unroll
     for (int k = 0; k < 17; ++k) c0[k] = c1[k] = cL[k] = 0;
-    Fe sum[3] = {fe_zero(), fe_zero(), fe_zero()};
     Fe sb0 = fe_zero(), sb1 = fe_zero();
     if (w.K) {
 #pragma unroll
@@ -534,7 +566,7 @@
             const uint64_t a = (uint64_t)(uintptr_t)fp.in[f] + w.r0 * 2048;
             glds_rows2(a, a + hi_off, w.voff, w.my_lds + f * 4096);
         }
-        int since = 0, lazy = 0;
+        int since = 0;
         for (uint64_t k = 0; k < w.K; ++k) {
             const bool last = k + 1 == w.K;
             const uint64_t next = (w.r0 + (k + 1) * w.rs) * 2048;
@@ -571,26 +603,15 @@
                 sb0 = fe_add(sb0, lo, P);
                 sb1 = fe_add(sb1, hi, P);
             }
-            ++lazy;
-            if (++since == 7 || lazy == kMaxLazy || last) {
+            if (++since == 7 || last) {
                 dot29_normalise(c0);
                 dot29_normalise(c1);
                 dot29_normalise(cL);
                 since = 0;
             }
-            if (lazy == kMaxLazy || last) {
-                dot29_flush(c0, sum[0], P);
-                dot29_flush(c1, sum[1], P);
-                dot29_flush(cL, sum[2], P);
-                lazy = 0;
-            }
-        }
-    }
-    if (EXTRA) {
-        sum[0] = fe_add(sum[0], sb0, P);
-        sum[1] = fe_add(sum[1], sb1, P);
-    }
-    block_reduce_store<3>(sum, partials, P);
+        }
+    }
+    dot29_block_store<EXTRA>(c0, c1, cL, sb0, sb1, partials);
 }
 template <int EXTRA>
 __global__ __launch_bounds__(kBlock, 2) void k_round0_glds(FactorPtrs fp, uint64_t q, FieldParams P, uint64_t *__restrict__ partials) {
@@ -663,11 +684,10 @@
     const Mul29 r = load_challenge29(rptr);
     asm volatile("s_waitcnt vmcnt(0)" ::: "memory");
     const GldsWave w = glds_wave(q, nblk);
-    Fe prod[NS], sum[NS], sum_b[NS];
+    Fe prod[NS], sum_b[NS];
     WideAcc acc[NS];
 #pragma unroll
     for (int t = 0; t < NS; ++t) {
-        sum[t] = fe_zero();
         sum_b[t] = fe_zero();
         wide_zero(acc[t]);
     }
@@ -685,16 +705,13 @@
             if constexpr (K + EXTRA > 2) fused_glds_unit<2, K, EXTRA, STORE_NT>(w, fp, q, run, last, r, P, prod, acc, sum_b);
             if constexpr (K + EXTRA > 3) fused_glds_unit<3, K, EXTRA, STORE_NT>(w, fp, q, run, last, r, P, prod, acc, sum_b);
         }
-#pragma unroll
-        for (int t = 0; t < NS; ++t)
-            if (t != 1) sum[t] = redc_wide(acc[t], P);
         if (EXTRA) {
 #pragma unroll
             for (int t = 0; t < K; ++t)
-                if (t != 1) sum[t] = fe_add(sum[t], sum_b[t], P);
-        }
-    }
-    block_reduce_store<NS, true>(sum, partials, P);
+                if (t != 1) wide_add_fe_hi(acc[t], sum_b[t]);
+        }
+    }
+    block_reduce_store_wide<NS, true>(acc, partials);
 }
 template <int K, int EXTRA, bool STORE_NT>
 __global__ __launch_bounds__(kBlock, 2) void k_round_fused_glds(FactorPtrs fp, uint64_t q, FieldParams P, const uint64_t *__restrict__ rptr,
@@ -770,41 +787,63 @@
         if constexpr (EXTRA) sum = fe_add(sum, w[K], P);
         j = jn;
     }
-    Fe s = sum;
-    if constexpr (K > 1) s = fe_add(redc_wide(acc, P), sum, P);
-    {
-        Fe a, b;
-#pragma unroll
-        for (int i = 0; i < 8; ++i) {
-            const auto x = __builtin_amdgcn_permlane32_swap(s.v[i], s.v[i], false, false);
-            a.v[i] = x[0];
-            b.v[i] = x[1];
-        }
-        s = fe_add(a, b, P);
-#pragma unroll
-        for (int i = 0; i < 8; ++i) {
-            const auto x = __builtin_amdgcn_permlane16_swap(s.v[i], s.v[i], false, false);
-            a.v[i] = x[0];
-            b.v[i] = x[1];
-        }
-        s = fe_add(a, b, P);
-        s = fe_add(s, fe_dpp<0x128>(s), P);
-        s = fe_add(s, fe_dpp<0x12C>(s), P);
-    }
-    if (lane < 4) {
-#pragma unroll
-        for (int i = 0; i < 8; ++i) red[wave][lane][i] = s.v[i];
-    }
-    __syncthreads();
-    if (threadIdx.x < (uint32_t)NS) {
-        Fe tot = fe_zero();
-        for (int wv = 0; wv < kBlock / 64; ++wv) {
-            Fe o;
-#pragma unroll
-            for (int i = 0; i < 8; ++i) o.v[i] = red[wv][threadIdx.x][i];
-            tot = fe_add(tot, o, P);
-        }
-        fe_store(partials, (uint64_t)blockIdx.x * NS + threadIdx.x, tot);
+    if constexpr (K > 1) {
+        __shared__ uint32_t redw[kBlock / 64][4][17];
+        if constexpr (EXTRA) wide_add_fe_hi(acc, sum);
+        wide_wave_sum<true>(acc);
+        if (lane < 4) {
+#pragma unroll
+            for (int i = 0; i < 17; ++i) redw[wave][lane][i] = acc.v[i];
+        }
+        __syncthreads();
+        if (threadIdx.x < (uint32_t)NS) {
+            WideAcc tot;
+#pragma unroll
+            for (int i = 0; i < 17; ++i) tot.v[i] = redw[0][threadIdx.x][i];
+            for (int wv = 1; wv < kBlock / 64; ++wv) {
+                WideAcc o;
+#pragma unroll
+                for (int i = 0; i < 17; ++i) o.v[i] = redw[wv][threadIdx.x][i];
+                wide_add(tot, o);
+            }
+            wide_store(partials, (uint64_t)blockIdx.x * NS + threadIdx.x, tot);
+        }
+    } else {
+        Fe s = sum;
+        {
+            Fe a, b;
+#pragma unroll
+            for (int i = 0; i < 8; ++i) {
+                const auto x = __builtin_amdgcn_permlane32_swap(s.v[i], s.v[i], false, false);
+                a.v[i] = x[0];
+                b.v[i] = x[1];
+            }
+            s = fe_add(a, b, P);
+#pragma unroll
+            for (int i = 0; i < 8; ++i) {
+                const auto x = __builtin_amdgcn_permlane16_swap(s.v[i], s.v[i], false, false);
+                a.v[i] = x[0];
+                b.v[i] = x[1];
+            }
+            s = fe_add(a, b, P);
+            s = fe_add(s, fe_dpp<0x128>(s), P);
+            s = fe_add(s, fe_dpp<0x12C>(s), P);
+        }
+        if (lane < 4) {
+#pragma unroll
+            for (int i = 0; i < 8; ++i) red[wave][lane][i] = s.v[i];
+        }
+        __syncthreads();
+        if (threadIdx.x < (uint32_t)NS) {
+            Fe tot = fe_zero();
+            for (int wv = 0; wv < kBlock / 64; ++wv) {
+                Fe o;
+#pragma unroll
+                for (int i = 0; i < 8; ++i) o.v[i] = red[wv][threadIdx.x][i];
+                tot = fe_add(tot, o, P);
+            }
+            fe_store(partials, (uint64_t)blockIdx.x * NS + threadIdx.x, tot);
+        }
     }
 }
 template <int K, int D, int EXTRA>
diff --git a/zk_amd/csrc/rounds.hip b/zk_amd/csrc/rounds.hip
--- a/zk_amd/csrc/rounds.hip
+++ b/zk_amd/csrc/rounds.hip
@@ -70,6 +70,12 @@
     return (uint32_t)(b ? b : 1);
 }
 
+static inline uint32_t glds_round0_grid(uint64_t q, uint32_t g) {
+    const uint64_t need = ((q >> 6) + (uint64_t)(kBlock / 64) * kGldsRound0MaxRuns - 1) / ((uint64_t)(kBlock / 64) * kGldsRound0MaxRuns);
+    const uint32_t two_per_cu = g > 512 ? 512 : g;
+    return need > two_per_cu ? (uint32_t)need : two_per_cu;
+}
+
 static inline uint32_t claim_blocks(const RoundLaunchCtx &lc) { return lc.claim.out ? 1u : 0u; }
 
 thread_local BatchRecorder *g_batch = nullptr;
@@ -78,14 +84,19 @@
     return (uint32_t)K | ((uint32_t)D << 4) | ((uint32_t)FUSED << 8) | ((uint32_t)EXTRA << 9) | ((uint32_t)SKIP1 << 10) | ((uint32_t)LEAD << 11);
 }
 template <int K, int D, bool FUSED, int EXTRA = 0, bool SKIP1 = false, bool LEAD = false>
-static void go_kd(const RoundLaunchCtx &lc, const FactorPtrs &fp, uint64_t q, const uint64_t *d_r, uint32_t grid, const ClaimJob &cj = {}) {
-    const FieldParams *P = lc.P;
-    hipStream_t st = lc.stream;
-    uint64_t *part = lc.d_partials;
-    auto single = [=]() {
-        k_round_kd<K, D, FUSED, EXTRA, SKIP1, LEAD><<<grid, kBlock, 0, st>>>(fp, q, *P, d_r, part, cj);
-        return hipGetLastError();
-    };
+static void go_kd(const RoundLaunchCtx &lc, const FactorPtrs &fp, uint64_t q, const uint64_t *d_r, uint32_t grid, const ClaimJob &cj = {},
+                  uint32_t wide_rec = 0) {
+    const FieldParams *P = lc.P;
+    hipStream_t st = lc.stream;
+    uint64_t *part = lc.d_partials;
+    auto single = [=]() {
+        k_round_kd<K, D, FUSED, EXTRA, SKIP1, LEAD><<<grid, kBlock, 0, st>>>(fp, q, *P, d_r, part, cj, wide_rec);
+        return hipGetLastError();
+    };
+    if (wide_rec) {
+        if (!batch_record_other(single)) (void)single();
+        return;
+    }
     if (batch_record(BK_ROUND_KD, kd_shape(K, D, FUSED, EXTRA, SKIP1, LEAD), grid, kBlock, 0, q, 0, 0, 0, RoundSlot{factor_ptrs4(fp), d_r, part, cj}, single))
         return;
     (void)single();
@@ -135,36 +146,40 @@
 }
 
 template <int K, int D>
-static void launch_kd(const RoundLaunchCtx &lc, const FactorPtrs &fp, uint64_t q, bool fused, const uint64_t *d_r, uint32_t g) {
-    if (fused) go_kd<K, D, true>(lc, fp, q, d_r, g);
-    else go_kd<K, D, false>(lc, fp, q, d_r, g);
+static void launch_kd(const RoundLaunchCtx &lc, const FactorPtrs &fp, uint64_t q, bool fused, const uint64_t *d_r, uint32_t g, uint32_t wide_rec = 0) {
+    if (fused) go_kd<K, D, true>(lc, fp, q, d_r, g, {}, wide_rec);
+    else go_kd<K, D, false>(lc, fp, q, d_r, g, {}, wide_rec);
 }
 template <int D>
-static void launch_generic(const RoundLaunchCtx &lc, const FactorPtrs &fp, int k, uint64_t q, bool fused, const uint64_t *d_r, uint32_t g) {
-    const FieldParams *P = lc.P;
-    hipStream_t st = lc.stream;
-    uint64_t *part = lc.d_partials;
-    auto single = [=]() {
-        if (fused) k_round<D, true><<<g, kBlock, 0, st>>>(fp, k, q, *P, d_r, part);
-        else k_round<D, false><<<g, kBlock, 0, st>>>(fp, k, q, *P, d_r, part);
+static void launch_generic(const RoundLaunchCtx &lc, const FactorPtrs &fp, int k, uint64_t q, bool fused, const uint64_t *d_r, uint32_t g,
+                           uint32_t wide_rec) {
+    const FieldParams *P = lc.P;
+    hipStream_t st = lc.stream;
+    uint64_t *part = lc.d_partials;
+    auto single = [=]() {
+        if (fused) k_round<D, true><<<g, kBlock, 0, st>>>(fp, k, q, *P, d_r, part, wide_rec);
+        else k_round<D, false><<<g, kBlock, 0, st>>>(fp, k, q, *P, d_r, part, wide_rec);
         return hipGetLastError();
     };
     if (!batch_record_other(single)) (void)single();
 }
 
 int launch_round(const RoundLaunchCtx &lc, const FactorPtrs &fp, int k, uint64_t q, uint32_t D, bool fused,
-                 const uint64_t *d_r, uint32_t *out_grid, bool *skip1, bool *lead) {
+                 const uint64_t *d_r, uint32_t *out_grid, bool *skip1, bool *lead, bool *wide) {
     if (D < 1 || D > 4 || k < 1 || k > kMaxFactors) return kLaunchUnsupported;
     uint32_t g = round_grid(q);
-    bool no_lead = false;
+    bool no_lead = false, no_wide = false;
     if (!lead) lead = &no_lead;
+    if (!wide) wide = &no_wide;
+    const uint32_t force_wide = *wide ? 1u : 0u;
+    *wide = true;
     if (*lead && !((k == 2 && D == 2) || (k == 3 && D == 3))) *lead = false;
     if (*lead && (uint64_t)g * (D + 1) <= lc.capacity_elems) {
         const int shl = k * 10 + (int)D;
         bool done = true;
         if (!fused) {
             if (shl == 22 && round0_dot29() && glds_takes(q, (uint64_t)1 << 21)) {
-                if (g > 512) g = 512;
+                g = glds_round0_grid(q, g);
                 go_round0_glds<0>(lc, fp, q, g);
             } else if (shl == 22 && round0_dot29()) go_round0_dot29<0>(lc, fp, q, g);
             else if (shl == 22) go_kd<2, 2, false, 0, false, true>(lc, fp, q, d_r, g);
@@ -211,8 +226,8 @@
     const bool fits = (uint64_t)g * (D + 1) <= lc.capacity_elems;
     const int shape = fits ? k * 10 + (int)D : 0;
     switch (shape) {
-        case 11: launch_kd<1, 1>(lc, fp, q, fused, d_r, g); break;
-        case 12: launch_kd<1, 2>(lc, fp, q, fused, d_r, g); break;
+        case 11: launch_kd<1, 1>(lc, fp, q, fused, d_r, g, force_wide); *wide = force_wide; break;
+        case 12: launch_kd<1, 2>(lc, fp, q, fused, d_r, g, force_wide); *wide = force_wide; break;
         case 21: launch_kd<2, 1>(lc, fp, q, fused, d_r, g); break;
         case 22: launch_kd<2, 2>(lc, fp, q, fused, d_r, g); break;
         case 23: launch_kd<2, 3>(lc, fp, q, fused, d_r, g); break;
@@ -220,11 +235,12 @@
         case 33: launch_kd<3, 3>(lc, fp, q, fused, d_r, g); break;
         default:
             g = capped_grid(q);
+            *wide = force_wide;
             switch (D) {
-                case 1: launch_generic<1>(lc, fp, k, q, fused, d_r, g); break;
-                case 2: launch_generic<2>(lc, fp, k, q, fused, d_r, g); break;
-                case 3: launch_generic<3>(lc, fp, k, q, fused, d_r, g); break;
-                default: launch_generic<4>(lc, fp, k, q, fused, d_r, g); break;
+                case 1: launch_generic<1>(lc, fp, k, q, fused, d_r, g, force_wide); break;
+                case 2: launch_generic<2>(lc, fp, k, q, fused, d_r, g, force_wide); break;
+                case 3: launch_generic<3>(lc, fp, k, q, fused, d_r, g, force_wide); break;
+                default: launch_generic<4>(lc, fp, k, q, fused, d_r, g, force_wide); break;
             }
     }
     if (hipGetLastError() != hipSuccess) return kLaunchHipError;
@@ -233,17 +249,19 @@
 }
 
 int launch_round_plus1(const RoundLaunchCtx &lc, const FactorPtrs &fp, int k, uint64_t q, uint32_t D, bool fused,
-                       const uint64_t *d_r, uint32_t *out_grid, bool *skip1, bool *lead) {
+                       const uint64_t *d_r, uint32_t *out_grid, bool *skip1, bool *lead, bool *wide) {
     uint32_t g = round_grid(q, min_blocks_plus1());
     if ((uint64_t)g * (D + 1) > lc.capacity_elems) return kLaunchUnsupported;
     const int shape = k * 10 + (int)D;
+    if (shape != 22 && shape != 33) return kLaunchUnsupported;
+    if (wide) *wide = true;
     bool no_lead = false;
     if (!lead) lead = &no_lead;
     if (*lead && shape == 22 && (!fused || (skip1 && *skip1))) {
         if (!fused) {
             if (round0_dot29_extra()) go_round0_dot29<1>(lc, fp, q, g);
             else if (round0_dot29() && glds_takes(q, (uint64_t)1 << 20)) {
-                if (g > 512) g = 512;
+                g = glds_round0_grid(q, g);
                 go_round0_glds<1>(lc, fp, q, g);
             } else go_kd<2, 2, false, 1, false, true>(lc, fp, q, d_r, g);
             if (skip1) *skip1 = false;
```
